# hmmlillian/Neural-Color-Transfer

Measured on AMD Instinct MI355X. Metric: 700x700 pairs/sec end-to-end L=5->1; PatchMatch HBM GB/s vs peak, higher is better.
Workload: dtype f32

## Files before the change

### neural-color-transfer_amd/csrc/k_wls_mg.hip

```cpp
#include "nct_internal.h"
#include <chrono>
#include <atomic>
#include <cstdlib>
#include <cstdio>
#include <cmath>
#include "nct_device.h"
#include <vector>
#include <cstring>
#include <string>
#include <thread>
#include <cstdarg>

namespace {
#ifndef NCT_MG_NS
#define NCT_MG_NS 3
#endif
constexpr int MG_NS = NCT_MG_NS;
static_assert(MG_NS >= 2 && MG_NS <= 4, "2, 3 or 4 smoothing sweeps per leg");
constexpr double MG_W[4] = {MG_NS == 2 ? 0.5808 : (MG_NS == 3 ? 0.5346 : 0.5193), MG_NS == 2 ? 2.6437 : (MG_NS == 3 ? 0.9677 : 0.7153), MG_NS == 3 ? 5.0974 : 1.5340, 8.0502};
constexpr double OMEGA = MG_W[0];
__host__ __device__ constexpr float mg_rk(int k) { return (float)(MG_W[k] / MG_W[0]); }
constexpr float MG_R0 = (float)(0.8 / MG_W[0]);
constexpr int NQMAX = 6;
#ifndef NCT_MG_TXB
#define NCT_MG_TXB 32
#define NCT_MG_TYB 16
#endif

typedef float vf;
struct Lvl { int H, W, n, nine;
             double *d, *wE, *wS, *wSE, *wSW, *pa, *pb;
             vf *fd, *fdinv, *fE, *fS, *fSE, *fSW;
             vf *fpst, *fpw;
             vf *b, *x, *x2;
             vf *lxm, *lxp, *lym, *lyp; };

struct PState { double gam[6], alp[6], bb[6]; int active[6]; int iters[6]; int nactive; int seq; double rho[6]; };

template <int NV>
__device__ __forceinline__ void mg_block_reduce(double (&v)[NV], double* __restrict__ partial, int lb = -1 ) {
    __shared__ double s_red[128 * NV];
    const int t = threadIdx.x;
    if (t >= 128) {
#pragma unroll
        for (int q = 0; q < NV; ++q) s_red[q * 128 + t - 128] = v[q];
    }
    __syncthreads();
    if (t < 128) {
#pragma unroll
        for (int q = 0; q < NV; ++q) v[q] += s_red[q * 128 + t];
    }
    __syncthreads();
    if (t >= 64 && t < 128) {
#pragma unroll
        for (int q = 0; q < NV; ++q) s_red[q * 128 + t - 64] = v[q];
    }
    __syncthreads();
    if (t < 64) {
#pragma unroll
        for (int q = 0; q < NV; ++q) {
            double x = v[q] + s_red[q * 128 + t];
            x += __shfl_down(x, 32); x += __shfl_down(x, 16); x += __shfl_down(x, 8);
            x += __shfl_down(x, 4); x += __shfl_down(x, 2); x += __shfl_down(x, 1);
            if (t == 0) partial[(size_t)(lb < 0 ? (int)blockIdx.x : lb) * NV + q] = x;
        }
    }
}
template <int NV>
__device__ __forceinline__ void mg_final_reduce(const double* __restrict__ partial, int nb, double (&out)[NV]) {
    __shared__ double s_fin[256 * NV];
    const int t = threadIdx.x;
    double acc[NV];
#pragma unroll
    for (int q = 0; q < NV; ++q) acc[q] = 0.0;
    for (int b = t; b < nb; b += 256)
#pragma unroll
        for (int q = 0; q < NV; ++q) acc[q] += partial[(size_t)b * NV + q];
#pragma unroll
    for (int q = 0; q < NV; ++q) s_fin[q * 256 + t] = acc[q];
    __syncthreads();
    for (int off = 128; off >= 1; off >>= 1) {
        if (t < off)
#pragma unroll
            for (int q = 0; q < NV; ++q) s_fin[q * 256 + t] += s_fin[q * 256 + t + off];
        __syncthreads();
    }
#pragma unroll
    for (int q = 0; q < NV; ++q) out[q] = s_fin[q * 256];
    __syncthreads();
}

template <int NV>
__device__ __forceinline__ void mg_final_reduce_strided(const double* __restrict__ partial, int nb, int stride, double (&out)[NV]) {
    __shared__ double s_fin2[256 * NV];
    const int t = threadIdx.x;
    double acc[NV];
#pragma unroll
    for (int q = 0; q < NV; ++q) acc[q] = 0.0;
    for (int b = t; b < nb; b += 256)
#pragma unroll
        for (int q = 0; q < NV; ++q) acc[q] += partial[(size_t)b * stride + q];
#pragma unroll
    for (int q = 0; q < NV; ++q) s_fin2[q * 256 + t] = acc[q];
    __syncthreads();
    for (int off = 128; off >= 1; off >>= 1) {
        if (t < off)
#pragma unroll
            for (int q = 0; q < NV; ++q) s_fin2[q * 256 + t] += s_fin2[q * 256 + t + off];
        __syncthreads();
    }
#pragma unroll
    for (int q = 0; q < NV; ++q) out[q] = s_fin2[q * 256];
    __syncthreads();
}

template <int NQ, typename F>
__device__ __forceinline__ void lvl_op(const Lvl& L, int i, F&& val , double (&y)[NQ]) {
    const int W = L.W, H = L.H;
    const int r = i / W, c = i - r * W;
    const double d = L.d[i];
    const bool e0 = c + 1 < W, e1 = c > 0, e2 = r + 1 < H, e3 = r > 0;
    const int j0 = e0 ? i + 1 : i, j1 = e1 ? i - 1 : i, j2 = e2 ? i + W : i, j3 = e3 ? i - W : i;
    const double w0 = L.wE[i], w1 = L.wE[j1], w2 = L.wS[i], w3 = L.wS[j3];
    double v0[NQ], v1[NQ], v2[NQ], v3[NQ];
#pragma unroll
    for (int q = 0; q < NQ; ++q) { y[q] = val(i, q); v0[q] = val(j0, q); v1[q] = val(j1, q); v2[q] = val(j2, q); v3[q] = val(j3, q); }
#pragma unroll
    for (int q = 0; q < NQ; ++q) {
        double t = d * y[q];
        t = e0 ? t - w0 * v0[q] : t;
        t = e1 ? t - w1 * v1[q] : t;
        t = e2 ? t - w2 * v2[q] : t;
        t = e3 ? t - w3 * v3[q] : t;
        y[q] = t;
    }
}

__device__ __forceinline__ int nb_dy(int k) { return k == 2 || k == 4 || k == 5 ? 1 : (k == 3 || k == 6 || k == 7 ? -1 : 0); }
__device__ __forceinline__ int nb_dx(int k) { return k == 0 || k == 4 || k == 6 ? 1 : (k == 1 || k == 5 || k == 7 ? -1 : 0); }
__device__ __forceinline__ unsigned nb_mask(const Lvl& L, int r, int c) {
    const bool xr = c + 1 < L.W, xl = c > 0, yd = r + 1 < L.H, yu = r > 0;
    unsigned m = (xr ? 1u : 0u) | (xl ? 2u : 0u) | (yd ? 4u : 0u) | (yu ? 8u : 0u);
    if (L.nine) m |= (xr && yd ? 16u : 0u) | (xl && yd ? 32u : 0u) | (xr && yu ? 64u : 0u) | (xl && yu ? 128u : 0u);
    return m;
}
__device__ __forceinline__ void coup8(const Lvl& L, int r, int c, double (&w)[8]) {
    const int W = L.W, i = r * W + c;
    const unsigned m = nb_mask(L, r, c);
    w[0] = (m & 1u) ? L.wE[i] : 0.0; w[1] = (m & 2u) ? L.wE[i - 1] : 0.0; w[2] = (m & 4u) ? L.wS[i] : 0.0; w[3] = (m & 8u) ? L.wS[i - W] : 0.0;
    w[4] = (m & 16u) ? L.wSE[i] : 0.0; w[5] = (m & 32u) ? L.wSW[i] : 0.0; w[6] = (m & 64u) ? L.wSW[i - W + 1] : 0.0; w[7] = (m & 128u) ? L.wSE[i - W - 1] : 0.0;
}
__global__ void k_mg_diag(Lvl L, const double* __restrict__ rough) {
    const int i = blockIdx.x * blockDim.x + threadIdx.x;
    if (i >= L.n) return;
    const int y = i / L.W, x = i - y * L.W;
    double a00 = 0.0;
    a00 += rough[i];
    if (x + 1 < L.W) a00 += L.wE[i];
    if (x > 0) a00 += L.wE[i - 1];
    if (y + 1 < L.H) a00 += L.wS[i];
    if (y > 0) a00 += L.wS[i - L.W];
    L.d[i] = a00;
    L.fd[i] = (vf)a00; L.fdinv[i] = (vf)(OMEGA / a00); L.fE[i] = (vf)L.wE[i]; L.fS[i] = (vf)L.wS[i];
}
__device__ __forceinline__ void mg_weights_at(const Lvl& L, int i) {
    const int r = i / L.W, c = i - r * L.W;
    double w[8]; coup8(L, r, c, w);
    const double d = L.d[i];
    double pa = 0.0, pb = 0.0;
    if (!(r & 1) && (c & 1)) { const double den = (d - w[2]) - w[3]; const bool e2 = c + 1 < L.W;
                               if (den > 0.0) { pa = ((w[1] + w[5]) + w[7]) / den; pb = ((w[0] + w[4]) + w[6]) / den; } else { pa = e2 ? 0.5 : 1.0; pb = e2 ? 0.5 : 0.0; } }
    else if ((r & 1) && !(c & 1)) { const double den = (d - w[0]) - w[1]; const bool e2 = r + 1 < L.H;
                                    if (den > 0.0) { pa = ((w[3] + w[6]) + w[7]) / den; pb = ((w[2] + w[4]) + w[5]) / den; } else { pa = e2 ? 0.5 : 1.0; pb = e2 ? 0.5 : 0.0; } }
    else if ((r & 1) && (c & 1)) pa = 1.0 / d;
    L.pa[i] = pa; L.pb[i] = pb;
}
__global__ void k_mg_weights(Lvl L) {
    const int i = blockIdx.x * blockDim.x + threadIdx.x;
    if (i >= L.n) return;
    mg_weights_at(L, i);
}
__device__ __forceinline__ void mg_pstencil_at(const Lvl& L, const Lvl& C, double* pst_out, int I) {
    const int Y = I / C.W, X = I - Y * C.W;
    const int W = L.W, H = L.H, r = 2 * Y, c = 2 * X, f = r * W + c;
    double pst[9];
#pragma unroll
    for (int k = 0; k < 9; ++k) pst[k] = 0.0;
    pst[4] = 1.0;
    if (c > 0) pst[3] = L.pb[f - 1];
    if (c + 1 < W) pst[5] = L.pa[f + 1];
    if (r > 0) pst[1] = L.pb[f - W];
    if (r + 1 < H) pst[7] = L.pa[f + W];
#pragma unroll
    for (int dy = -1; dy <= 1; dy += 2)
#pragma unroll
        for (int dx = -1; dx <= 1; dx += 2) {
            const int y = r + dy, x = c + dx;
            if (y < 0 || y >= H || x < 0 || x >= W) continue;
            double w[8]; coup8(L, y, x, w);
            const double wdiag = dy < 0 ? (dx < 0 ? w[4] : w[5]) : (dx < 0 ? w[6] : w[7]);
            const double wvert = dy < 0 ? w[2] : w[3];
            const double whor = dx < 0 ? w[0] : w[1];
            pst[(dy + 1) * 3 + dx + 1] = ((wdiag + wvert * pst[3 + dx + 1]) + whor * pst[(dy + 1) * 3 + 1]) * L.pa[y * W + x];
        }
#pragma unroll
    for (int k = 0; k < 9; ++k) { pst_out[(size_t)I * 9 + k] = pst[k]; L.fpst[(size_t)I * 9 + k] = (vf)pst[k]; }
}
__global__ void k_mg_pstencil(Lvl L, Lvl C, double* __restrict__ pst_out) {
    const int I = blockIdx.x * blockDim.x + threadIdx.x;
    if (I >= C.n) return;
    mg_pstencil_at(L, C, pst_out, I);
}
__device__ __forceinline__ void mg_pweights_at(const Lvl& L, const Lvl& C, int i) {
    const int r = i / L.W, c = i - r * L.W;
    const int Y0 = r >> 1, X0 = c >> 1, ny = (r & 1) ? 2 : 1, nx = (c & 1) ? 2 : 1;
    vf pw[4] = {0.f, 0.f, 0.f, 0.f};
    if (ny * nx > 1) {
        int sl = 0;
        for (int jy = 0; jy < ny; ++jy)
            for (int jx = 0; jx < nx; ++jx, ++sl) {
                const int Y = Y0 + jy, X = X0 + jx;
                if (Y < C.H && X < C.W) pw[sl] = L.fpst[(size_t)(Y * C.W + X) * 9 + (r - 2 * Y + 1) * 3 + (c - 2 * X + 1)];
            }
    }
#pragma unroll
    for (int k = 0; k < 4; ++k) L.fpw[(size_t)k * L.n + i] = pw[k];
}
__global__ void k_mg_pweights(Lvl L, Lvl C) {
    const int i = blockIdx.x * blockDim.x + threadIdx.x;
    if (i >= L.n) return;
    mg_pweights_at(L, C, i);
}
__device__ __forceinline__ void mg_galerkin_at(const Lvl& L, const Lvl& C, const double* pst, int I) {
    const int Wc = C.W, Hc = C.H, Y = I / Wc, X = I - Y * Wc;
    const int W = L.W, H = L.H;
    const int JY[5] = {0, 0, 1, 1, 1}, JX[5] = {0, 1, 0, 1, -1};
    bool jok[5]; double acc[5];
#pragma unroll
    for (int j = 0; j < 5; ++j) { const int yj = Y + JY[j], xj = X + JX[j]; jok[j] = yj < Hc && xj >= 0 && xj < Wc; acc[j] = 0.0; }
    const double* pI = pst + (size_t)I * 9;
    for (int dy = -1; dy <= 1; ++dy)
        for (int dx = -1; dx <= 1; ++dx) {
            const int y = 2 * Y + dy, x = 2 * X + dx;
            if (y < 0 || y >= H || x < 0 || x >= W) continue;
            const double pi = pI[(dy + 1) * 3 + dx + 1];
            double w[8]; coup8(L, y, x, w);
            const unsigned m = nb_mask(L, y, x);
            const double di = L.d[y * W + x];
#pragma unroll
            for (int j = 0; j < 5; ++j) {
                if (!jok[j]) continue;
                const double* pJ = pst + (size_t)(I + JY[j] * Wc + JX[j]) * 9;
                const int ry = dy - 2 * JY[j], rx = dx - 2 * JX[j];
                double au = (ry >= -1 && ry <= 1 && rx >= -1 && rx <= 1) ? di * pJ[(ry + 1) * 3 + rx + 1] : 0.0;
#pragma unroll
                for (int k = 0; k < 8; ++k) {
                    if (!(m & (1u << k))) continue;
                    const int ky = ry + nb_dy(k), kx = rx + nb_dx(k);
                    if (ky < -1 || ky > 1 || kx < -1 || kx > 1) continue;
                    au -= w[k] * pJ[(ky + 1) * 3 + kx + 1];
                }
                acc[j] += pi * au;
            }
        }
    C.d[I] = acc[0];
    C.wE[I] = jok[1] ? -acc[1] : 0.0;
    C.wS[I] = jok[2] ? -acc[2] : 0.0;
    C.wSE[I] = jok[3] ? -acc[3] : 0.0;
    C.wSW[I] = jok[4] ? -acc[4] : 0.0;
}
__global__ void k_mg_galerkin(Lvl L, Lvl C, const double* __restrict__ pst) {
    const int I = blockIdx.x * blockDim.x + threadIdx.x;
    if (I >= C.n) return;
    mg_galerkin_at(L, C, pst, I);
}
__device__ __forceinline__ void mg_finish_at(const Lvl& L, int i) {
    const int r = i / L.W, c = i - r * L.W;
    const double d = L.d[i];
    double w[8]; coup8(L, r, c, w);
    double s = fabs(d);
#pragma unroll
    for (int k = 0; k < 8; ++k) s += fabs(w[k]);
    const double h = 0.5 * s, dt = h > d ? h : d;
    L.fd[i] = (vf)d; L.fdinv[i] = (vf)(OMEGA / dt); L.fE[i] = (vf)L.wE[i]; L.fS[i] = (vf)L.wS[i]; L.fSE[i] = (vf)L.wSE[i]; L.fSW[i] = (vf)L.wSW[i];
}
__global__ void k_mg_finish(Lvl L) {
    const int i = blockIdx.x * blockDim.x + threadIdx.x;
    if (i >= L.n) return;
    mg_finish_at(L, i);
}

#ifndef NCT_MG_TAIL_N
#define NCT_MG_TAIL_N 512
#endif
constexpr int MG_TAIL_N = NCT_MG_TAIL_N;
constexpr int MG_MAXL = 12;
struct LvlPack { Lvl lv[MG_MAXL]; };
__global__ __launch_bounds__(1024) void k_mg_setup_tail(LvlPack P, int l0, int nl, double* pst) {
    const int t = threadIdx.x;
    for (int l = l0; l < nl; ++l) {
        const Lvl& L = P.lv[l - 1]; const Lvl& C = P.lv[l];
        for (int I = t; I < C.n; I += 1024) mg_pstencil_at(L, C, pst, I);
        __syncthreads();
        for (int i = t; i < L.n; i += 1024) mg_pweights_at(L, C, i);
        for (int I = t; I < C.n; I += 1024) mg_galerkin_at(L, C, pst, I);
        __syncthreads();
        for (int i = t; i < C.n; i += 1024) mg_finish_at(C, i);
        if (l + 1 < nl) {
            for (int i = t; i < C.n; i += 1024) mg_weights_at(C, i);
        }
        __syncthreads();
    }
}

struct PxCoef { vf d, dinv, w[8]; unsigned ex; };
template <bool NINE>
__device__ __forceinline__ PxCoef px_coef(const Lvl& L, int gy, int gx) {
    const int i = gy * L.W + gx, W = L.W;
    PxCoef c;
    const bool xr = gx + 1 < W, xl = gx > 0, yd = gy + 1 < L.H, yu = gy > 0;
    c.ex = (xr ? 1u : 0u) | (xl ? 2u : 0u) | (yd ? 4u : 0u) | (yu ? 8u : 0u);
    c.d = L.fd[i]; c.dinv = L.fdinv[i];
    c.w[0] = xr ? L.fE[i] : 0.f; c.w[1] = xl ? L.fE[i - 1] : 0.f; c.w[2] = yd ? L.fS[i] : 0.f; c.w[3] = yu ? L.fS[i - W] : 0.f;
    if (NINE) {
        c.ex |= (xr && yd ? 16u : 0u) | (xl && yd ? 32u : 0u) | (xr && yu ? 64u : 0u) | (xl && yu ? 128u : 0u);
        c.w[4] = (xr && yd) ? L.fSE[i] : 0.f; c.w[5] = (xl && yd) ? L.fSW[i] : 0.f; c.w[6] = (xr && yu) ? L.fSW[i - W + 1] : 0.f; c.w[7] = (xl && yu) ? L.fSE[i - W - 1] : 0.f;
    } else { c.w[4] = c.w[5] = c.w[6] = c.w[7] = 0.f; }
    return c;
}
template <int LW> __device__ __forceinline__ constexpr int lds_off(int k) {
    return k == 0 ? 1 : k == 1 ? -1 : k == 2 ? LW : k == 3 ? -LW : k == 4 ? LW + 1 : k == 5 ? LW - 1 : k == 6 ? -LW + 1 : -LW - 1;
}
template <int NQ, int LW, int LN, bool NINE>
__device__ __forceinline__ void lds_op(const PxCoef& c, const vf* __restrict__ s_v, int p, const vf (&own)[NQ], vf (&y)[NQ]) {
#pragma unroll
    for (int q = 0; q < NQ; ++q) y[q] = c.d * own[q];
#pragma unroll
    for (int k = 0; k < (NINE ? 8 : 4); ++k)
        if (c.ex & (1u << k)) {
#pragma unroll
            for (int q = 0; q < NQ; ++q) y[q] -= c.w[k] * s_v[q * LN + p + lds_off<LW>(k)];
        }
}
__device__ __forceinline__ int mg_tile_of_block(int bid, int ntiles) {
    const int q = ntiles >> 3, r = ntiles & 7, xcd = bid & 7, idx = bid >> 3;
    return (xcd < r ? xcd * (q + 1) : r * (q + 1) + (xcd - r) * q) + idx;
}
constexpr int mg_threads(int TX, int TY, bool X0 = false) { return ((TX + 2 * MG_NS + 1 + (X0 ? 2 : 0)) * (TY + 2 * MG_NS + 1 + (X0 ? 2 : 0)) + 63) / 64 * 64; }
template <int NQ, int TX, int TY, typename TB, bool NINE, bool X0 = false>
__global__ __launch_bounds__(mg_threads(TX, TY, X0)) void k_mg_down(const PState* __restrict__ st, Lvl F, const TB* __restrict__ b, vf* __restrict__ x, Lvl C, vf* __restrict__ bc, const vf* __restrict__ x1 = nullptr) {
    const int nact = st->nactive;
    constexpr int S0 = X0 ? 1 : 0;
    constexpr int HA = MG_NS + 1 + S0, HB = MG_NS + S0, LW = TX + HA + HB, LH = TY + HA + HB, LN = LW * LH;
    static_assert(LN <= mg_threads(TX, TY, X0) && mg_threads(TX, TY, X0) <= 1024, "one thread per pixel of the tile and its halo");
    __shared__ vf s_a[NQ * LN], s_b[NQ * LN];
    const int tiles_x = (F.W + TX - 1) / TX, tile = mg_tile_of_block(blockIdx.x, gridDim.x);
    const int x0 = (tile % tiles_x) * TX, y0 = (tile / tiles_x) * TY;
    const int p = threadIdx.x;
    const int ly = p / LW, lx = p - ly * LW;
    const int gy = y0 + ly - HA, gx = x0 + lx - HA;
    const bool valid = p < LN && gy >= 0 && gy < F.H && gx >= 0 && gx < F.W;
    auto ring = [&](int k) { return valid && lx >= k && lx <= LW - 1 - k && ly >= k && ly <= LH - 1 - k; };
    const bool interior = valid && lx >= HA && lx < HA + TX && ly >= HA && ly < HA + TY;
    const bool coarse = interior && !(gy & 1) && !(gx & 1);
    const int i = gy * F.W + gx;
    vf bq[NQ], xk[NQ], ps[9]; PxCoef c;
    if (valid) {
        c = px_coef<NINE>(F, gy, gx);
        if (coarse) {
            const vf* pp = F.fpst + (size_t)((gy >> 1) * C.W + (gx >> 1)) * 9;
#pragma unroll
            for (int k = 0; k < 9; ++k) ps[k] = pp[k];
        }
#pragma unroll
        for (int q = 0; q < NQ; ++q) { bq[q] = (vf)b[(size_t)q * F.n + i]; xk[q] = X0 ? x1[(size_t)q * F.n + i] : bq[q] * c.dinv; s_a[q * LN + p] = xk[q]; }
    }
    if (nact == 0) return;
    __syncthreads();
#pragma unroll
    for (int k = 1 - S0; k < MG_NS; ++k) {
        vf* src = ((k + S0) & 1) ? s_a : s_b; vf* dst = ((k + S0) & 1) ? s_b : s_a;
        if (ring(k + S0)) {
            vf y[NQ]; lds_op<NQ, LW, LN, NINE>(c, src, p, xk, y);
#pragma unroll
            for (int q = 0; q < NQ; ++q) {
                xk[q] = xk[q] + (bq[q] - y[q]) * (k == 0 ? c.dinv : c.dinv * mg_rk(k));
                dst[q * LN + p] = xk[q];
                if (k == MG_NS - 1 && interior) x[(size_t)q * F.n + i] = xk[q];
            }
        }
        __syncthreads();
    }
    vf* xs = ((MG_NS + S0) & 1) ? s_a : s_b; vf* rs = ((MG_NS + S0) & 1) ? s_b : s_a;
    if (ring(MG_NS + S0)) {
        vf yv[NQ]; lds_op<NQ, LW, LN, NINE>(c, xs, p, xk, yv);
#pragma unroll
        for (int q = 0; q < NQ; ++q) rs[q * LN + p] = bq[q] - yv[q];
    }
    __syncthreads();
    if (coarse) {
        const bool xr = (c.ex & 1u) != 0, xl = (c.ex & 2u) != 0, yd = (c.ex & 4u) != 0, yu = (c.ex & 8u) != 0;
        const bool in[9] = {xl && yu, yu, xr && yu, xl, true, xr, xl && yd, yd, xr && yd};
        vf acc[NQ];
#pragma unroll
        for (int q = 0; q < NQ; ++q) acc[q] = 0.0f;
#pragma unroll
        for (int k = 0; k < 9; ++k)
            if (in[k]) {
#pragma unroll
                for (int q = 0; q < NQ; ++q) acc[q] += ps[k] * rs[q * LN + p + (k / 3 - 1) * LW + (k % 3 - 1)];
            }
#pragma unroll
        for (int q = 0; q < NQ; ++q) bc[(size_t)q * C.n + (gy >> 1) * C.W + (gx >> 1)] = acc[q];
    }
}
template <int NQ, int TX, int TY, typename TB, bool NINE>
__global__ __launch_bounds__(mg_threads(TX, TY)) void k_mg_up(const PState* __restrict__ st, Lvl L, const TB* __restrict__ b, const vf* __restrict__ x, int Wc, int nc,
                                                              const vf* __restrict__ ec, vf* __restrict__ xo) {
    const int nact = st->nactive;
    constexpr bool ODD = (MG_NS & 1) != 0;
    constexpr int HA = ODD ? MG_NS + 1 : MG_NS, HB = ODD ? MG_NS : MG_NS + 1, LW = TX + HA + HB, LH = TY + HA + HB, LN = LW * LH;
    constexpr int OL = ODD ? 1 : 0, OR = ODD ? 0 : 1;
    __shared__ vf s_a[NQ * LN], s_b[NQ * LN];
    const int tiles_x = (L.W + TX - 1) / TX, tile = mg_tile_of_block(blockIdx.x, gridDim.x);
    const int x0 = (tile % tiles_x) * TX, y0 = (tile / tiles_x) * TY;
    const int p = threadIdx.x;
    const int ly = p / LW, lx = p - ly * LW;
    const int gy = y0 + ly - HA, gx = x0 + lx - HA;
    const bool valid = p < LN && gy >= 0 && gy < L.H && gx >= 0 && gx < L.W;
    auto ring = [&](int k) { return valid && lx >= OL + k && lx <= LW - 1 - OR - k && ly >= OL + k && ly <= LH - 1 - OR - k; };
    const bool oy = (gy & 1) != 0, ox = (gx & 1) != 0;
    const int i = gy * L.W + gx;
    vf bq[NQ], xk[NQ], pw[4]; PxCoef c;
    if (valid) {
        c = px_coef<NINE>(L, gy, gx);
#pragma unroll
        for (int k = 0; k < 4; ++k) pw[k] = L.fpw[(size_t)k * L.n + i];
#pragma unroll
        for (int q = 0; q < NQ; ++q) { bq[q] = (vf)b[(size_t)q * L.n + i]; xk[q] = x[(size_t)q * L.n + i]; }
        if (!oy && !ox) {
            const int ip = (gy >> 1) * Wc + (gx >> 1);
#pragma unroll
            for (int q = 0; q < NQ; ++q) s_a[q * LN + p] = ec[(size_t)q * nc + ip];
        }
    }
    if (nact == 0) return;
    __syncthreads();
    if (ring(0)) {
        const bool xr = (c.ex & 1u) != 0, yd = (c.ex & 4u) != 0;
        const int o0 = -(oy ? LW : 0) - (ox ? 1 : 0);
        const int o1 = (oy && ox) ? -LW + 1 : (ox ? 1 : LW);
        const bool e1 = (oy && ox) ? xr : (ox ? xr : yd);
        const bool e2 = oy && ox && yd, e3 = oy && ox && yd && xr;
        const bool copy = !oy && !ox;
        const int a1 = e1 ? o1 : o0, a2 = e2 ? LW - 1 : o0, a3 = e3 ? LW + 1 : o0;
        vf v0[NQ], v1[NQ], v2[NQ], v3[NQ];
#pragma unroll
        for (int q = 0; q < NQ; ++q) { v0[q] = s_a[q * LN + p + (copy ? 0 : o0)]; v1[q] = s_a[q * LN + p + (copy ? 0 : a1)]; v2[q] = s_a[q * LN + p + (copy ? 0 : a2)]; v3[q] = s_a[q * LN + p + (copy ? 0 : a3)]; }
#pragma unroll
        for (int q = 0; q < NQ; ++q) {
            vf e = pw[0] * v0[q];
            e = e1 ? e + pw[1] * v1[q] : e;
            e = e2 ? e + pw[2] * v2[q] : e;
            e = e3 ? e + pw[3] * v3[q] : e;
            e = copy ? v0[q] : e;
            xk[q] = xk[q] + e; s_b[q * LN + p] = xk[q];
        }
    }
    __syncthreads();
#pragma unroll
    for (int k = 0; k < MG_NS; ++k) {
        vf* src = (k & 1) ? s_a : s_b; vf* dst = (k & 1) ? s_b : s_a;
        if (ring(k + 1)) {
            vf y[NQ]; lds_op<NQ, LW, LN, NINE>(c, src, p, xk, y);
#pragma unroll
            for (int q = 0; q < NQ; ++q) {
                xk[q] = xk[q] + (bq[q] - y[q]) * (k == 0 ? c.dinv : c.dinv * mg_rk(k));
                if (k == MG_NS - 1) xo[(size_t)q * L.n + i] = xk[q]; else dst[q * LN + p] = xk[q];
            }
        }
        if (k < MG_NS - 1) __syncthreads();
    }
}
constexpr int LBX = 32, LBY = 16, LBP = LBX + 1, LBN = LBY * LBP + 1;
constexpr float LINE_OM = 0.9f;
__global__ void k_mg_lines_setup(Lvl L) {
    const int t = blockIdx.x * blockDim.x + threadIdx.x;
    const int W = L.W, H = L.H, nbx = (W + LBX - 1) / LBX, nby = (H + LBY - 1) / LBY;
    if (t < H * nbx) {
        const int r = t / nbx, c0 = (t - r * nbx) * LBX;
        double p = 0.0;
        for (int c = c0; c < W && c < c0 + LBX; ++c) {
            const int i = r * W + c;
            if (c == c0) { p = L.d[i]; L.lxm[i] = 0.0f; }
            else { const double w = L.wE[i - 1], m = w / p; p = L.d[i] - w * m; L.lxm[i] = (vf)m; }
            L.lxp[i] = (vf)(1.0 / p);
        }
    } else if (t < H * nbx + W * nby) {
        const int u = t - H * nbx, c = u / nby, r0 = (u - c * nby) * LBY;
        double p = 0.0;
        for (int r = r0; r < H && r < r0 + LBY; ++r) {
            const int i = r * W + c;
            if (r == r0) { p = L.d[i]; L.lym[i] = 0.0f; }
            else { const double w = L.wS[i - W], m = w / p; p = L.d[i] - w * m; L.lym[i] = (vf)m; }
            L.lyp[i] = (vf)(1.0 / p);
        }
    }
}
template <int LEN, int STR>
__device__ __forceinline__ void line_solve(const vf* __restrict__ s_r, vf* __restrict__ s_e, const vf* __restrict__ s_m, const vf* __restrict__ s_p, const vf* __restrict__ s_w, int len) {
    vf y[LEN];
    if (len == LEN) {
        constexpr int CH = 8;
        static_assert(LEN % CH == 0, "line length");
#pragma unroll
        for (int k = 0; k < LEN; ++k) y[k] = s_r[k * STR];
        vf t = 0.0f;
#pragma unroll
        for (int k0 = 0; k0 < LEN; k0 += CH) {
            vf m[CH];
#pragma unroll
            for (int j = 0; j < CH; ++j) m[j] = s_m[(k0 + j) * STR];
#pragma unroll
            for (int j = 0; j < CH; ++j) { const int k = k0 + j; if (k == 0) t = y[0]; else { t = y[k] + m[j] * t; y[k] = t; } }
        }
#pragma unroll
        for (int k0 = LEN - CH; k0 >= 0; k0 -= CH) {
            vf pp[CH], ww[CH];
#pragma unroll
            for (int j = 0; j < CH; ++j) { pp[j] = s_p[(k0 + j) * STR]; ww[j] = s_w[(k0 + j) * STR]; }
#pragma unroll
            for (int j = CH - 1; j >= 0; --j) { const int k = k0 + j; t = k == LEN - 1 ? y[k] * pp[j] : (y[k] + ww[j] * t) * pp[j]; y[k] = t; }
        }
#pragma unroll
        for (int k = 0; k < LEN; ++k) s_e[k * STR] = y[k];
        return;
    }
#pragma unroll
    for (int k = 0; k < LEN; ++k) if (k < len) y[k] = s_r[k * STR];
    vf t = y[0];
#pragma unroll
    for (int k = 1; k < LEN; ++k) if (k < len) { t = y[k] + s_m[k * STR] * t; y[k] = t; }
#pragma unroll
    for (int k = LEN - 1; k >= 0; --k)
        if (k < len) {
            if (k == len - 1) t = y[k] * s_p[k * STR];
            else t = (y[k] + s_w[k * STR] * t) * s_p[k * STR];
            s_e[k * STR] = t;
        }
}
template <int NQ, bool POST>
__global__ __launch_bounds__(LBX * LBY, 8) void k_mg_block(const PState* __restrict__ st, Lvl L, const vf* __restrict__ b, const vf* __restrict__ xin, vf* __restrict__ xout) {
    const int nact = st->nactive;
    constexpr int XW = LBX + 2, XN = XW * (LBY + 2);
    static_assert(NQ * XN <= (NQ + 6) * LBN, "the halo tile of the iterate lives where e1 and the factors go afterwards");
    __shared__ vf s_all[(2 * NQ + 6) * LBN];
    vf* const s_r = s_all; vf* const s_e1 = s_all + NQ * LBN; vf* const s_x = s_e1;
    vf* const s_xm = s_all + 2 * NQ * LBN; vf* const s_xp = s_xm + LBN; vf* const s_xw = s_xp + LBN; vf* const s_ym = s_xw + LBN; vf* const s_yp = s_ym + LBN; vf* const s_yw = s_yp + LBN;
    const int W = L.W, H = L.H, nbx = (W + LBX - 1) / LBX;
    const int blk = mg_tile_of_block(blockIdx.x, gridDim.x);
    const int x0 = (blk % nbx) * LBX, y0 = (blk / nbx) * LBY;
    const int bw = x0 + LBX <= W ? LBX : W - x0, bh = y0 + LBY <= H ? LBY : H - y0;
    const int p = threadIdx.x, ly = p / LBX, lx = p - ly * LBX, gy = y0 + ly, gx = x0 + lx;
    const bool valid = ly < bh && lx < bw;
    const int i = gy * W + gx, lp = ly * LBP + lx;
    vf own[NQ], bq[NQ];
    if (POST) {
        for (int h = p; h < XN; h += LBX * LBY) {
            const int hy = h / XW, hx = h - hy * XW, yy = y0 + hy - 1, xx = x0 + hx - 1;
            if (yy >= 0 && yy < H && xx >= 0 && xx < W) {
#pragma unroll
                for (int q = 0; q < NQ; ++q) s_x[q * XN + h] = xin[(size_t)q * L.n + yy * W + xx];
            }
        }
    }
    vf fE_own = 0.f, fS_own = 0.f, c_xm = 0.f, c_xp = 0.f, c_ym = 0.f, c_yp = 0.f;
    if (valid) {
        c_xm = L.lxm[i]; c_xp = L.lxp[i]; c_ym = L.lym[i]; c_yp = L.lyp[i]; fE_own = L.fE[i]; fS_own = L.fS[i];
#pragma unroll
        for (int q = 0; q < NQ; ++q) bq[q] = b[(size_t)q * L.n + i];
    }
    if (nact == 0) return;
    if (POST) {
        __syncthreads();
        if (valid) {
            const vf d = L.fd[i];
            const bool xr = gx + 1 < W, xl = gx > 0, yd = gy + 1 < H, yu = gy > 0;
            const vf wW = xl ? L.fE[i - 1] : 0.f, wN = yu ? L.fS[i - W] : 0.f;
            const int hp = (ly + 1) * XW + lx + 1;
#pragma unroll
            for (int q = 0; q < NQ; ++q) {
                own[q] = s_x[q * XN + hp];
                const vf vE = s_x[q * XN + hp + 1], vW = s_x[q * XN + hp - 1], vS = s_x[q * XN + hp + XW], vN = s_x[q * XN + hp - XW];
                vf y = d * own[q];
                y = xr ? y - fE_own * vE : y;
                y = xl ? y - wW * vW : y;
                y = yd ? y - fS_own * vS : y;
                y = yu ? y - wN * vN : y;
                bq[q] = bq[q] - y;
            }
        }
        __syncthreads();
    }
    if (valid) {
        s_xm[lp] = c_xm; s_xp[lp] = c_xp; s_ym[lp] = c_ym; s_yp[lp] = c_yp; s_xw[lp] = fE_own; s_yw[lp] = fS_own;
#pragma unroll
        for (int q = 0; q < NQ; ++q) s_r[q * LBN + lp] = bq[q];
    }
    __syncthreads();
    if (!POST) { if (p < LBY * NQ) { const int row = p % LBY, q = p / LBY; if (row < bh) { const int o = row * LBP; line_solve<LBX, 1>(s_r + q * LBN + o, s_e1 + q * LBN + o, s_xm + o, s_xp + o, s_xw + o, bw); } } }
    else       { if (p < LBX * NQ) { const int col = p % LBX, q = p / LBX; if (col < bw) line_solve<LBY, LBP>(s_r + q * LBN + col, s_e1 + q * LBN + col, s_ym + col, s_yp + col, s_yw + col, bh); } }
    __syncthreads();
    if (valid) {
#pragma unroll
        for (int q = 0; q < NQ; ++q) {
            vf acc = 0.0f;
            if (!POST) { if (ly + 1 < bh) acc += fS_own * s_e1[q * LBN + lp + LBP]; if (ly > 0) acc += s_yw[lp - LBP] * s_e1[q * LBN + lp - LBP]; }
            else       { if (lx + 1 < bw) acc += fE_own * s_e1[q * LBN + lp + 1];   if (lx > 0) acc += s_xw[lp - 1] * s_e1[q * LBN + lp - 1]; }
            s_r[q * LBN + lp] = acc;
        }
    }
    __syncthreads();
    if (!POST) { if (p < LBX * NQ) { const int col = p % LBX, q = p / LBX; if (col < bw) line_solve<LBY, LBP>(s_r + q * LBN + col, s_r + q * LBN + col, s_ym + col, s_yp + col, s_yw + col, bh); } }
    else       { if (p < LBY * NQ) { const int row = p % LBY, q = p / LBY; if (row < bh) { const int o = row * LBP; line_solve<LBX, 1>(s_r + q * LBN + o, s_r + q * LBN + o, s_xm + o, s_xp + o, s_xw + o, bw); } } }
    __syncthreads();
    if (valid) {
#pragma unroll
        for (int q = 0; q < NQ; ++q) {
            const vf u = (s_e1[q * LBN + lp] + s_r[q * LBN + lp]) * LINE_OM;
            xout[(size_t)q * L.n + i] = POST ? own[q] + u : u;
        }
    }
}

#ifndef NCT_MID_MAXP0
#define NCT_MID_MAXP0 2
#endif
static_assert(NCT_MID_MAXP0 == 1 || NCT_MID_MAXP0 == 2, "k_mg_mid is instantiated for one or two pixels per thread at its first level (four measured slower: DESIGN.md 9)");
constexpr int MID_T = 1024, MID_P1 = 1, MID_N1 = MID_T * MID_P1, MID_LV = 5;
constexpr int mid_cap(int d) { return d == 1 ? 1024 : (d == 2 ? 256 : 64); }
constexpr int mid_stash_off(int d) { return d <= 1 ? 0 : mid_stash_off(d - 1) + 14 * mid_cap(d - 1); }
constexpr int MID_STASH = mid_stash_off(MID_LV);
constexpr int mid_ppt(int P0, int D) { return D == 0 ? P0 : (D == 1 ? MID_P1 : 1); }
struct MidPack { Lvl lv[MID_LV]; int nl; };
__device__ __forceinline__ vf mid_op(const PxCoef& c, const vf* __restrict__ s_v, int i, int W, vf* centre = nullptr) {
    const vf v0 = s_v[i];
    if (centre) *centre = v0;
    vf y = c.d * v0;
    vf t[8];
#pragma unroll
    for (int k = 0; k < 8; ++k) t[k] = s_v[(c.ex & (1u << k)) ? i + nb_dy(k) * W + nb_dx(k) : i];
#pragma unroll
    for (int k = 0; k < 8; ++k) y -= c.w[k] * ((c.ex & (1u << k)) ? t[k] : 0.0f);
    return y;
}
__device__ __forceinline__ vf mid_restrict(const vf* __restrict__ s_res, const vf (&ps)[9], int I, int Wc, int Wf, int Hf) {
    const int Y = I / Wc, X = I - Y * Wc, r = 2 * Y, c = 2 * X;
    vf acc = 0.0f, t[9]; bool in[9];
#pragma unroll
    for (int k = 0; k < 9; ++k) {
        const int yy = r + k / 3 - 1, xx = c + k % 3 - 1;
        in[k] = yy >= 0 && yy < Hf && xx >= 0 && xx < Wf;
        t[k] = s_res[in[k] ? yy * Wf + xx : r * Wf + c];
    }
#pragma unroll
    for (int k = 0; k < 9; ++k) acc = in[k] ? acc + ps[k] * t[k] : acc;
    return acc;
}
__device__ __forceinline__ vf mid_prolong(const vf* __restrict__ s_c, const vf (&pw)[4], int gy, int gx, int Wc, int Hc) {
    const int Y0 = gy >> 1, X0 = gx >> 1;
    const bool oy = (gy & 1) != 0, ox = (gx & 1) != 0;
    const bool xr = X0 + 1 < Wc, yd = Y0 + 1 < Hc;
    const int i00 = Y0 * Wc + X0, i01 = xr ? i00 + 1 : i00, i10 = yd ? i00 + Wc : i00, i11 = (yd && xr) ? i00 + Wc + 1 : i00;
    const vf c00 = s_c[i00], c01 = s_c[i01], c10 = s_c[i10], c11 = s_c[i11];
    if (!oy && !ox) return c00;
    vf e = pw[0] * c00;
    if (oy && ox) {
        e = xr ? e + pw[1] * c01 : e;
        e = yd ? e + pw[2] * c10 : e;
        e = (yd && xr) ? e + pw[3] * c11 : e;
    } else if (ox) { e = xr ? e + pw[1] * c01 : e; }
    else { e = yd ? e + pw[1] * c10 : e; }
    return e;
}
template <int P0, int D>
__device__ __forceinline__ void mid_level(const MidPack& P, int q, int t, vf* __restrict__ sA, vf* __restrict__ sB, vf* __restrict__ sC, vf* __restrict__ sS,
                                          const vf (&breg)[mid_ppt(P0, D)], int sweeps) {
    constexpr int PPT = mid_ppt(P0, D);
    const Lvl& L = P.lv[D];
    const int n = L.n, W = L.W;
    if (D == P.nl - 1) {
        if (t < n) sA[t] = breg[0];
        __syncthreads();
        if (t < 64) {
            const int i = t;
            const bool live = i < n;
            const int r = live ? i / W : 0, c = live ? i - r * W : 0;
            vf bq = 0.f, d = 0.f, dv = 0.f, w[8]; unsigned ex = 0;
#pragma unroll
            for (int k = 0; k < 8; ++k) w[k] = 0.f;
            if (live) { const PxCoef pc = px_coef<true>(L, r, c); d = pc.d; dv = pc.dinv; ex = pc.ex; bq = sA[i];
#pragma unroll
                for (int k = 0; k < 8; ++k) w[k] = pc.w[k]; }
            vf x = 0.0f;
            for (int s = 0; s < sweeps; ++s) {
                vf y = d * x;
#pragma unroll
                for (int k = 0; k < 8; ++k) {
                    const vf xn = __shfl(x, (i + nb_dy(k) * W + nb_dx(k)) & 63);
                    if (ex & (1u << k)) y -= w[k] * xn;
                }
                if (live) x = x + (bq - y) * (dv * MG_R0);
            }
            if (live) { if (D == 0) L.x2[(size_t)q * n + i] = x; else sC[i] = x; }
        }
        __syncthreads();
        return;
    }
    if constexpr (D + 1 < MID_LV) {
        const Lvl& C = P.lv[D + 1];
        constexpr int CPT = mid_ppt(P0, D + 1);
        vf* __restrict__ stash = sS + mid_stash_off(D);
        vf x[PPT];
        {
            PxCoef c[PPT]; vf ps[CPT][9];
#pragma unroll
            for (int k = 0; k < PPT; ++k) { const int i = t + k * MID_T; if (i < n) c[k] = px_coef<true>(L, i / W, i % W); }
#pragma unroll
            for (int k = 0; k < CPT; ++k) { const int I = t + k * MID_T; if (I < C.n) {
#pragma unroll
                for (int j = 0; j < 9; ++j) ps[k][j] = L.fpst[(size_t)I * 9 + j]; } }
            if constexpr (D >= 1) {
                if (t < n) {
                    vf pw[4];
#pragma unroll
                    for (int j = 0; j < 4; ++j) pw[j] = L.fpw[(size_t)j * n + t];
                    stash[t] = c[0].d; stash[n + t] = c[0].dinv;
#pragma unroll
                    for (int j = 0; j < 8; ++j) stash[(2 + j) * n + t] = c[0].w[j];
#pragma unroll
                    for (int j = 0; j < 4; ++j) stash[(10 + j) * n + t] = pw[j];
                }
            }
#pragma unroll
            for (int k = 0; k < PPT; ++k) { const int i = t + k * MID_T; if (i < n) sA[i] = breg[k] * c[k].dinv; }
            __syncthreads();
#pragma unroll
            for (int sw = 1; sw < MG_NS; ++sw) {
                vf* src = (sw & 1) ? sA : sB; vf* dst = (sw & 1) ? sB : sA;
#pragma unroll
                for (int k = 0; k < PPT; ++k) {
                    const int i = t + k * MID_T;
                    if (i < n) {
                        vf xs; const vf y = mid_op(c[k], src, i, W, &xs);
                        const vf xv = xs + (breg[k] - y) * (c[k].dinv * mg_rk(sw));
                        dst[i] = xv;
                        if (sw == MG_NS - 1) x[k] = xv;
                    }
                }
                __syncthreads();
            }
            {
                vf* xs = (MG_NS & 1) ? sA : sB; vf* rs = (MG_NS & 1) ? sB : sA;
#pragma unroll
                for (int k = 0; k < PPT; ++k) { const int i = t + k * MID_T; if (i < n) rs[i] = breg[k] - mid_op(c[k], xs, i, W); }
            }
            __syncthreads();
            vf bc[CPT];
#pragma unroll
            for (int k = 0; k < CPT; ++k) { const int I = t + k * MID_T; bc[k] = I < C.n ? mid_restrict((MG_NS & 1) ? sB : sA, ps[k], I, C.W, W, L.H) : 0.f; }
            __syncthreads();
            asm volatile("" ::: "memory");
            mid_level<P0, D + 1>(P, q, t, sA, sB, sC, sS, bc, sweeps);
        }
        PxCoef c[PPT]; vf pw[PPT][4];
        if constexpr (D == 0) {
#pragma unroll
            for (int k = 0; k < PPT; ++k) { const int i = t + k * MID_T; if (i < n) { c[k] = px_coef<true>(L, i / W, i % W);
#pragma unroll
                for (int j = 0; j < 4; ++j) pw[k][j] = L.fpw[(size_t)j * n + i]; } }
        } else {
            if (t < n) {
                const int gy = t / W, gx = t - gy * W;
                const bool xr = gx + 1 < W, xl = gx > 0, yd = gy + 1 < L.H, yu = gy > 0;
                c[0].ex = (xr ? 1u : 0u) | (xl ? 2u : 0u) | (yd ? 4u : 0u) | (yu ? 8u : 0u) | (xr && yd ? 16u : 0u) | (xl && yd ? 32u : 0u) | (xr && yu ? 64u : 0u) | (xl && yu ? 128u : 0u);
                c[0].d = stash[t]; c[0].dinv = stash[n + t];
#pragma unroll
                for (int j = 0; j < 8; ++j) c[0].w[j] = stash[(2 + j) * n + t];
#pragma unroll
                for (int j = 0; j < 4; ++j) pw[0][j] = stash[(10 + j) * n + t];
            }
        }
#pragma unroll
        for (int k = 0; k < PPT; ++k) {
            const int i = t + k * MID_T;
            if (i < n) sA[i] = x[k] + mid_prolong(sC, pw[k], i / W, i % W, C.W, C.H);
        }
        __syncthreads();
#pragma unroll
        for (int sw = 0; sw < MG_NS; ++sw) {
            vf* src = (sw & 1) ? sB : sA; vf* dst = (sw & 1) ? sA : sB;
#pragma unroll
            for (int k = 0; k < PPT; ++k) {
                const int i = t + k * MID_T;
                if (i < n) {
                    vf xs; const vf y = mid_op(c[k], src, i, W, &xs);
                    const vf v = xs + (breg[k] - y) * (sw == 0 ? c[k].dinv : c[k].dinv * mg_rk(sw));
                    if (sw < MG_NS - 1) dst[i] = v;
                    else if (D == 0) L.x2[(size_t)q * n + i] = v; else sC[i] = v;
                }
            }
            __syncthreads();
        }
    }
}
template <int P0>
__global__ __launch_bounds__(MID_T) void k_mg_mid(const PState* __restrict__ st, MidPack P, int sweeps) {
    const int nact = st->nactive;
    __shared__ vf sA[MID_T * P0], sB[MID_T * P0], sC[MID_N1], sS[MID_STASH];
    const int q = blockIdx.x, t = threadIdx.x;
    const Lvl& L0 = P.lv[0];
    vf b[P0];
#pragma unroll
    for (int k = 0; k < P0; ++k) { const int i = t + k * MID_T; b[k] = i < L0.n ? L0.b[(size_t)q * L0.n + i] : 0.f; }
    if (nact == 0) return;
    mid_level<P0, 0>(P, q, t, sA, sB, sC, sS, b, sweeps);
}


__device__ __forceinline__ void pcg_publish(PState* __restrict__ host_out, const PState& v, int seq) {
    PState o = v; o.seq = 0;
    *host_out = o;
    __threadfence_system();
    __hip_atomic_store(&host_out->seq, seq, __ATOMIC_RELEASE, __HIP_MEMORY_SCOPE_SYSTEM);
}
template <int NQ>
__global__ __launch_bounds__(256) void k_pcg_start(Lvl L, const double* __restrict__ rough, const double* __restrict__ X , double* __restrict__ x6, double* __restrict__ r, vf* __restrict__ rf, double* __restrict__ partial) {
    const int i = blockIdx.x * 256 + threadIdx.x;
    double acc[2 * NQ];
#pragma unroll
    for (int q = 0; q < 2 * NQ; ++q) acc[q] = 0.0;
    if (i < L.n) {
        auto xv = [&](int j, int q) { return X[((size_t)(q / 3) * L.n + j) * 3 + (q % 3)]; };
        double y[NQ]; lvl_op<NQ>(L, i, xv, y);
        const double rg = rough[i];
#pragma unroll
        for (int q = 0; q < NQ; ++q) {
            const double x0 = xv(i, q);
            const double bq = rg * x0;
            const double rv = bq - y[q];
            x6[(size_t)q * L.n + i] = x0; r[(size_t)q * L.n + i] = rv; rf[(size_t)q * L.n + i] = (vf)rv;
            acc[q] = rv * rv; acc[NQ + q] = bq * bq;
        }
    }
    mg_block_reduce<2 * NQ>(acc, partial);
}
template <int NQ>
__global__ void k_pcg_start_fin(const double* __restrict__ partial, int nb, PState* __restrict__ st, double rtol2, PState* __restrict__ host_out, int seq) {
    double s[2 * NQ]; mg_final_reduce<2 * NQ>(partial, nb, s);
    if (threadIdx.x < NQ) { const int q = threadIdx.x; st->bb[q] = s[NQ + q]; st->gam[q] = 0; st->alp[q] = 0; st->iters[q] = 0; st->rho[q] = s[q];
                            st->active[q] = (s[q] > rtol2 * s[NQ + q]) ? 1 : 0; }
    __syncthreads();
    if (threadIdx.x == 0) { int na = 0; for (int q = 0; q < NQ; ++q) na += st->active[q]; st->nactive = na; if (host_out) pcg_publish(host_out, *st, seq); }
}
template <int NQ>
__global__ __launch_bounds__(256) void k_cg_apply(const PState* __restrict__ st, Lvl L, const vf* __restrict__ z, const double* __restrict__ r,
                                                  double* __restrict__ w, double* __restrict__ partial) {
    const int nact = st->nactive;
    const int lb = mg_tile_of_block(blockIdx.x, gridDim.x);
    const int i = lb * 256 + threadIdx.x;
    double acc[3 * NQ];
#pragma unroll
    for (int q = 0; q < 3 * NQ; ++q) acc[q] = 0.0;
    auto uv = [&](int j, int q) { return (double)z[(size_t)q * L.n + j]; };
    double y[NQ], rq[NQ], uq[NQ];
#pragma unroll
    for (int q = 0; q < NQ; ++q) { y[q] = 0.0; rq[q] = 0.0; uq[q] = 0.0; }
    if (i < L.n) {
        lvl_op<NQ>(L, i, uv, y);
#pragma unroll
        for (int q = 0; q < NQ; ++q) { rq[q] = r[(size_t)q * L.n + i]; uq[q] = uv(i, q); }
    }
    if (nact == 0) return;
    if (i < L.n) {
#pragma unroll
        for (int q = 0; q < NQ; ++q) {
            const double u = uq[q], rv = rq[q];
            w[(size_t)q * L.n + i] = y[q];
            acc[q] = rv * u; acc[NQ + q] = y[q] * u; acc[2 * NQ + q] = rv * rv;
        }
    }
    mg_block_reduce<3 * NQ>(acc, partial, lb);
}
template <int NQ>
__global__ void k_cg_fin(const PState* __restrict__ st, const double* __restrict__ partial, int nb, double* __restrict__ sums) {
    if (st->nactive == 0) return;
    double s[NQ]; mg_final_reduce_strided<NQ>(partial + blockIdx.x * NQ, nb, 3 * NQ, s);
    if (threadIdx.x < NQ) sums[blockIdx.x * NQ + threadIdx.x] = s[threadIdx.x];
}
template <int NQ>
__global__ __launch_bounds__(256) void k_cg_update(int n, const PState* __restrict__ sc, PState* __restrict__ sn, const double* __restrict__ sums, double rtol2, int first,
                                                   const vf* __restrict__ z, const double* __restrict__ w, double* __restrict__ p, double* __restrict__ s,
                                                   double* __restrict__ x, double* __restrict__ r, vf* __restrict__ rf, PState* __restrict__ host_out, int seq) {
    if (sc->nactive == 0) { if (blockIdx.x == 0 && threadIdx.x == 0) { *sn = *sc; if (host_out) pcg_publish(host_out, *sc, seq); } return; }
    double al[NQ], be[NQ]; bool act[NQ];
#pragma unroll
    for (int q = 0; q < NQ; ++q) {
        const double gam = sums[q], del = sums[NQ + q], rho = sums[2 * NQ + q];
        act[q] = sc->active[q] != 0 && rho > rtol2 * sc->bb[q];
        be[q] = first ? 0.0 : gam / sc->gam[q];
        al[q] = first ? gam / del : gam / (del - be[q] * gam / sc->alp[q]);
    }
    if (blockIdx.x == 0 && threadIdx.x == 0) {
        int na = 0;
#pragma unroll
        for (int q = 0; q < NQ; ++q) {
            sn->bb[q] = sc->bb[q];
            sn->gam[q] = act[q] ? sums[q] : sc->gam[q]; sn->alp[q] = act[q] ? al[q] : sc->alp[q];
            sn->iters[q] = sc->iters[q] + (act[q] ? 1 : 0); sn->active[q] = act[q] ? 1 : 0; na += act[q] ? 1 : 0;
            sn->rho[q] = sc->active[q] != 0 ? sums[2 * NQ + q] : sc->rho[q];
        }
        sn->nactive = na;
        if (host_out) pcg_publish(host_out, *sn, seq);
    }
    const int i = blockIdx.x * 256 + threadIdx.x;
    if (i >= n) return;
    vf zq[NQ]; double wq[NQ], pq[NQ], sq[NQ], xq[NQ], rq[NQ];
#pragma unroll
    for (int q = 0; q < NQ; ++q) {
        zq[q] = 0.f; wq[q] = pq[q] = sq[q] = xq[q] = rq[q] = 0.0;
        if (act[q]) {
            const size_t j = (size_t)q * n + i;
            zq[q] = z[j]; wq[q] = w[j]; xq[q] = x[j]; rq[q] = r[j];
            if (!first) { pq[q] = p[j]; sq[q] = s[j]; }
        }
    }
#pragma unroll
    for (int q = 0; q < NQ; ++q) {
        if (!act[q]) continue;
        const size_t j = (size_t)q * n + i;
        const double zv = (double)zq[q], wv = wq[q];
        const double pn = first ? zv : zv + be[q] * pq[q];
        const double sv = first ? wv : wv + be[q] * sq[q];
        p[j] = pn; s[j] = sv;
        x[j] = xq[q] + al[q] * pn;
        const double rn = rq[q] - al[q] * sv;
        r[j] = rn; rf[j] = (vf)rn;
    }
}
template <int NQ>
__global__ void k_pcg_finish(int n, const double* __restrict__ x6, double* __restrict__ X) {
    const int i = blockIdx.x * blockDim.x + threadIdx.x;
    if (i >= n * NQ) return;
    const int q = i / n, px = i - q * n;
    X[((size_t)(q / 3) * n + px) * 3 + (q % 3)] = x6[i];
}
}

#define LCHK() NCT_LAUNCH_CHECK()
#ifndef NCT_WLS_BATCH
#define NCT_WLS_BATCH 2
#endif

namespace {
struct ErrSink {
    std::string err;
    int fail(int code, const char* fmt, ...) { char buf[512]; va_list ap; va_start(ap, fmt); vsnprintf(buf, sizeof buf, fmt, ap); va_end(ap); err = buf; return code; }
};
static std::atomic<int> g_seq{0};
struct PartBufs {
    double *x6, *r, *p, *sv, *w, *partial, *sums; PState* st;
    vf* rf;
    std::vector<Lvl> lv;
    PState* hst;
    const double* rough;
    nct_ctx* kt;
    int maxit;
    bool trace;
    bool forecast;
    bool lines;
    int iters[NQMAX];
};
template <int NQ>
int pcg_part(ErrSink* ctx, hipStream_t s, double* X , PartBufs& B, double rtol) {
    const std::vector<Lvl>& lv = B.lv;
    const int nl = (int)lv.size();
    const Lvl& F = lv[0];
    const int N = F.n, nb = cdiv(N, 256);
    double *x6 = B.x6, *r = B.r, *p = B.p, *sv = B.sv, *w = B.w, *partial = B.partial, *sums = B.sums;
    vf* rf = B.rf;
    PState* st = B.st;
    const PState* cur = st;
    const double rtol2 = rtol * rtol;
    hipLaunchKernelGGL(k_pcg_start<NQ>, dim3(nb), dim3(256), 0, s, F, B.rough, (const double*)X, (double*)x6, (double*)r, rf, (double*)partial); LCHK();
    int seq_of_slot[2] = {0, 0};
    seq_of_slot[0] = ++g_seq;
    hipLaunchKernelGGL(k_pcg_start_fin<NQ>, dim3(1), dim3(256), 0, s, (const double*)partial, nb, st, rtol2, &B.hst[0], seq_of_slot[0]); LCHK();

    constexpr int TXB = NCT_MG_TXB, TYB = NCT_MG_TYB;
    auto down = [&](int l) {
        const dim3 gb(cdiv(lv[l].W, TXB) * cdiv(lv[l].H, TYB)), gs(cdiv(lv[l].W, 16) * cdiv(lv[l].H, 8));
        if (l == 0 && B.lines) {
            constexpr int TYL = TYB - 2;
            const dim3 gbl(cdiv(lv[0].W, TXB) * cdiv(lv[0].H, TYL));
            if (lv[l].n >= 100000) hipLaunchKernelGGL((k_mg_down<NQ, TXB, TYL, vf, false, true>), gbl, dim3(mg_threads(TXB, TYL, true)), 0, s, cur, lv[l], (const vf*)rf, lv[l].x, lv[l + 1], lv[l + 1].b, (const vf*)lv[0].x2);
            else                   hipLaunchKernelGGL((k_mg_down<NQ, 16, 8, vf, false, true>), gs, dim3(mg_threads(16, 8, true)), 0, s, cur, lv[l], (const vf*)rf, lv[l].x, lv[l + 1], lv[l + 1].b, (const vf*)lv[0].x2);
        } else if (l == 0) {
            if (lv[l].n >= 100000) hipLaunchKernelGGL((k_mg_down<NQ, TXB, TYB, vf, false>), gb, dim3(mg_threads(TXB, TYB)), 0, s, cur, lv[l], (const vf*)rf, lv[l].x, lv[l + 1], lv[l + 1].b);
            else                   hipLaunchKernelGGL((k_mg_down<NQ, 16, 8, vf, false>), gs, dim3(mg_threads(16, 8)), 0, s, cur, lv[l], (const vf*)rf, lv[l].x, lv[l + 1], lv[l + 1].b);
        } else {
            if (lv[l].n >= 100000) hipLaunchKernelGGL((k_mg_down<NQ, TXB, TYB, vf, true>), gb, dim3(mg_threads(TXB, TYB)), 0, s, cur, lv[l], (const vf*)lv[l].b, lv[l].x, lv[l + 1], lv[l + 1].b);
            else                   hipLaunchKernelGGL((k_mg_down<NQ, 16, 8, vf, true>), gs, dim3(mg_threads(16, 8)), 0, s, cur, lv[l], (const vf*)lv[l].b, lv[l].x, lv[l + 1], lv[l + 1].b);
        }
    };
    auto block_step = [&](bool post) {
        if (!B.lines) return;
        const dim3 gl(cdiv(lv[0].W, LBX) * cdiv(lv[0].H, LBY));
        if (!post) hipLaunchKernelGGL((k_mg_block<NQ, false>), gl, dim3(LBX * LBY), 0, s, cur, lv[0], (const vf*)rf, (const vf*)nullptr, lv[0].x2);
        else       hipLaunchKernelGGL((k_mg_block<NQ, true>), gl, dim3(LBX * LBY), 0, s, cur, lv[0], (const vf*)rf, (const vf*)lv[0].x2, lv[0].x);
    };
    auto up = [&](int l, const vf* ec) {
        const dim3 gb(cdiv(lv[l].W, TXB) * cdiv(lv[l].H, TYB)), gs(cdiv(lv[l].W, 16) * cdiv(lv[l].H, 8));
        const int Wc = lv[l + 1].W, nc = lv[l + 1].n;
        if (l == 0) {
            if (lv[l].n >= 100000) hipLaunchKernelGGL((k_mg_up<NQ, TXB, TYB, vf, false>), gb, dim3(mg_threads(TXB, TYB)), 0, s, cur, lv[l], (const vf*)rf, (const vf*)lv[l].x, Wc, nc, ec, lv[l].x2);
            else                   hipLaunchKernelGGL((k_mg_up<NQ, 16, 8, vf, false>), gs, dim3(mg_threads(16, 8)), 0, s, cur, lv[l], (const vf*)rf, (const vf*)lv[l].x, Wc, nc, ec, lv[l].x2);
        } else {
            if (lv[l].n >= 100000) hipLaunchKernelGGL((k_mg_up<NQ, TXB, TYB, vf, true>), gb, dim3(mg_threads(TXB, TYB)), 0, s, cur, lv[l], (const vf*)lv[l].b, (const vf*)lv[l].x, Wc, nc, ec, lv[l].x2);
            else                   hipLaunchKernelGGL((k_mg_up<NQ, 16, 8, vf, true>), gs, dim3(mg_threads(16, 8)), 0, s, cur, lv[l], (const vf*)lv[l].b, (const vf*)lv[l].x, Wc, nc, ec, lv[l].x2);
        }
    };
    int tail0 = nl - 1;
    auto mid_fits = [&](int first) {
        if (nl - first > MID_LV) return false;
        for (int l = first; l < nl; ++l) { const int d = l - first; if (lv[l].n > (d == 0 ? NCT_MID_MAXP0 * MID_T : mid_cap(d))) return false; }
        return true;
    };
    while (tail0 > 1 && mid_fits(tail0 - 1)) --tail0;
    MidPack pack; memset(&pack, 0, sizeof pack); pack.nl = nl - tail0;
    for (int l = tail0; l < nl; ++l) pack.lv[l - tail0] = lv[l];
    bool ktime = false;
    auto kt_b = [&](int id) -> int { if (ktime && B.kt->kt_begin(s, id)) return ctx->fail(NCT_ERR_HIP, "%s", B.kt->err.c_str()); return 0; };
    auto kt_e = [&]() -> int { if (ktime && B.kt->kt_end(s)) return ctx->fail(NCT_ERR_HIP, "%s", B.kt->err.c_str()); return 0; };
    auto vcycle = [&]() -> int {
        if (ktime) {
            if (B.lines) { NCT_TRY(kt_b(NCT_KT_WLS_BLOCK_PRE)); block_step(false); LCHK(); NCT_TRY(kt_e()); }
            NCT_TRY(kt_b(NCT_KT_WLS_DOWN)); down(0); LCHK(); NCT_TRY(kt_e());
            NCT_TRY(kt_b(NCT_KT_WLS_COARSE));
            for (int l = 1; l < tail0; ++l) { down(l); LCHK(); }
            if (lv[tail0].n <= MID_T) hipLaunchKernelGGL(k_mg_mid<1>, dim3(NQ), dim3(MID_T), 0, s, cur, pack, 60);
            else                      hipLaunchKernelGGL(k_mg_mid<2>, dim3(NQ), dim3(MID_T), 0, s, cur, pack, 60);
            LCHK();
            for (int l = tail0 - 1; l >= 1; --l) { up(l, lv[l + 1].x2); LCHK(); }
            NCT_TRY(kt_e());
            NCT_TRY(kt_b(NCT_KT_WLS_UP)); up(0, lv[1].x2); LCHK(); NCT_TRY(kt_e());
            if (B.lines) { NCT_TRY(kt_b(NCT_KT_WLS_BLOCK_POST)); block_step(true); LCHK(); NCT_TRY(kt_e()); }
            return 0;
        }
        block_step(false); LCHK();
        for (int l = 0; l < tail0; ++l) { down(l); LCHK(); }
        if (lv[tail0].n <= MID_T) hipLaunchKernelGGL(k_mg_mid<1>, dim3(NQ), dim3(MID_T), 0, s, cur, pack, 60);
        else                      hipLaunchKernelGGL(k_mg_mid<2>, dim3(NQ), dim3(MID_T), 0, s, cur, pack, 60);
        LCHK();
        for (int l = tail0 - 1; l >= 0; --l) { up(l, lv[l + 1].x2); LCHK(); }
        block_step(true); LCHK();
        return 0;
    };
    const vf* z = B.lines ? lv[0].x : lv[0].x2;
    const int maxit = B.maxit, batch = NCT_WLS_BATCH;
    PState* hst = B.hst;
    PState* pub_to = nullptr; int pub_seq = 0;
    auto iteration = [&](int it) -> int {
        cur = st + (it & 1);
        PState* nxt = st + ((it + 1) & 1);
        ktime = B.kt != nullptr && it >= 2 && it < 6 && tail0 >= 1;
        NCT_TRY(vcycle());
        NCT_TRY(kt_b(NCT_KT_WLS_APPLY));
        hipLaunchKernelGGL(k_cg_apply<NQ>, dim3(nb), dim3(256), 0, s, cur, F, z, (const double*)r, (double*)w, (double*)partial); LCHK();
        NCT_TRY(kt_e());
        hipLaunchKernelGGL(k_cg_fin<NQ>, dim3(3), dim3(256), 0, s, cur, (const double*)partial, nb, (double*)sums); LCHK();
        NCT_TRY(kt_b(NCT_KT_WLS_UPDATE));
        hipLaunchKernelGGL(k_cg_update<NQ>, dim3(nb), dim3(256), 0, s, N, cur, nxt, (const double*)sums, rtol2, it == 0 ? 1 : 0, z, (const double*)w,
                           (double*)p, (double*)sv, (double*)x6, (double*)r, rf, pub_to, pub_seq); LCHK();
        NCT_TRY(kt_e());
        cur = nxt;
        return 0;
    };
    auto wait_published = [&](int slot) -> int {
        const int want_seq = seq_of_slot[slot];
        const auto t0 = std::chrono::steady_clock::now();
        for (unsigned spins = 1; __atomic_load_n(&hst[slot].seq, __ATOMIC_ACQUIRE) != want_seq; ++spins) {
            if (spins > 4096) std::this_thread::yield();
            if ((spins & 0xFFFFu) == 0) {
                const hipError_t q = hipStreamQuery(s);
                if (q != hipSuccess && q != hipErrorNotReady) return ctx->fail(NCT_ERR_HIP, "WLS MG-PCG: stream error while polling the solver state: %s", hipGetErrorString(q));
                if (std::chrono::steady_clock::now() - t0 > std::chrono::seconds(60)) return ctx->fail(NCT_ERR_HIP, "WLS MG-PCG: the solver state was not published within 60 s");
            }
        }
        return 0;
    };
    int it = 0; bool done = false;
    int issued = 0, seen = -1;
    int its_at_snapshot[2] = {0, 0};
    PState fin; memset(&fin, 0, sizeof fin);
    double prev_rho[6]; int prev_its = -1;
    int remaining_after_seen = -1;
    int its_seen = 0;
    bool forecast_on = B.forecast;
    while (true) {
        int want = batch;
        if (forecast_on && remaining_after_seen >= 0) {
            const int inflight = it - its_seen;
            want = remaining_after_seen - inflight;
            if (want > batch) want = batch;
            if (want < 0) want = 0;
            if (want == 0 && issued == seen) { want = batch; forecast_on = false; }
        }
        if (it + want > maxit) want = maxit - it;
        if (want > 0) {
            for (int k = 0; k < want; ++k, ++it) {
                if (k == want - 1) { seq_of_slot[(issued + 1) & 1] = ++g_seq; pub_to = &hst[(issued + 1) & 1]; pub_seq = seq_of_slot[(issued + 1) & 1]; }
                int rc = iteration(it); pub_to = nullptr; if (rc) return rc;
            }
            ++issued; its_at_snapshot[issued & 1] = it;
        }
        if (seen == issued) break;
        ++seen;
        NCT_TRY(wait_published(seen & 1));
        fin = hst[seen & 1];
        its_seen = its_at_snapshot[seen & 1];
        if (fin.nactive == 0) { done = true; break; }
        if (it >= maxit && seen == issued) break;
        if (B.forecast) {
            const int ridx = its_seen > 0 ? its_seen - 1 : 0;
            int need = -1; bool ok = prev_its >= 0 && ridx > prev_its;
            if (ok) {
                need = 1;
                for (int q = 0; q < NQ; ++q) {
                    if (!fin.active[q]) continue;
                    const double thr = rtol2 * fin.bb[q], rho = fin.rho[q];
                    if (!(rho > 0.0) || !(prev_rho[q] > 0.0) || !(thr > 0.0)) { ok = false; break; }
                    const double decay = pow(rho / prev_rho[q], 1.0 / (double)(ridx - prev_its));
                    if (!(decay < 0.95)) { ok = false; break; }
                    const double m = rho * decay <= thr ? 1.0 : 1.0 + ceil(log(thr / (rho * decay)) / log(decay));
                    if (m > need) need = (int)(m < 1e6 ? m : 1e6);
                }
            }
            remaining_after_seen = ok ? need : -1;
            for (int q = 0; q < NQ; ++q) prev_rho[q] = fin.rho[q];
            prev_its = ridx;
        }
    }
    if (!done) return ctx->fail(NCT_ERR_HIP, "WLS MG-PCG did not converge in %d iterations", maxit);
    hipLaunchKernelGGL(k_pcg_finish<NQ>, dim3(cdiv(N * NQ, 256)), dim3(256), 0, s, N, (const double*)x6, X); LCHK();
    for (int q = 0; q < NQ; ++q) B.iters[q] = fin.iters[q];
    if (B.trace) {
        int mx = 0; for (int q = 0; q < NQ; ++q) mx = fin.iters[q] > mx ? fin.iters[q] : mx;
        fprintf(stderr, "nct wls: %d x %d, %d iterations enqueued, %d needed (+1 that finds every system converged), %d snapshots read\n", F.W, F.H, it, mx, seen + 1);
    }
    return 0;
}
}

int nctk_wls_solve_mg(nct_ctx* ctx, hipStream_t s, double* X, const double* rough, const double* wx, const double* wy, int H, int W,
                      double rtol, int* iters_out ) {
    const bool split = ctx->wls_split != 0;
    const int nq0 = split ? 3 : 6;
    std::vector<Lvl> lv;
    std::vector<void*> owned;
    struct Cleanup { nct_ctx* c; std::vector<void*>& v; ~Cleanup() { for (void* q : v) c->release(q); } } cleanup{ctx, owned};
    auto newd = [&](size_t n) -> double* { void* q = ctx->alloc(n * sizeof(double)); if (q) owned.push_back(q); return (double*)q; };
    auto newf = [&](size_t n) -> vf* { void* q = ctx->alloc(n * sizeof(vf)); if (q) owned.push_back(q); return (vf*)q; };
    {
        int h = H, w = W;
        for (int l = 0;; ++l) {
            Lvl L; memset(&L, 0, sizeof L); L.H = h; L.W = w; L.n = h * w; L.nine = l > 0 ? 1 : 0;
            const bool last = L.n <= 64 || (h <= 8 && w <= 8) || l >= 15;
            if (l == 0) { L.wE = (double*)wx; L.wS = (double*)wy; }
            else { L.wE = newd(L.n); L.wS = newd(L.n); L.wSE = newd(L.n); L.wSW = newd(L.n); L.fSE = newf(L.n); L.fSW = newf(L.n);
                   if (!L.wE || !L.wS || !L.wSE || !L.wSW || !L.fSE || !L.fSW) return NCT_ERR_HIP; }
            L.d = newd(L.n); L.fd = newf(L.n); L.fdinv = newf(L.n); L.fE = newf(L.n); L.fS = newf(L.n);
            if (!last) { L.pa = newd(L.n); L.pb = newd(L.n); }
            if (!last) { L.fpst = newf((size_t)((h + 1) / 2) * ((w + 1) / 2) * 9); L.fpw = newf((size_t)L.n * 4); }
            L.b = l == 0 ? nullptr : newf((size_t)L.n * nq0); L.x = newf((size_t)L.n * nq0); L.x2 = newf((size_t)L.n * nq0);
            if (l == 0 && ctx->wls_lines) { L.lxm = newf(L.n); L.lxp = newf(L.n); L.lym = newf(L.n); L.lyp = newf(L.n); if (!L.lxm || !L.lxp || !L.lym || !L.lyp) return NCT_ERR_HIP; }
            if (!L.d || !L.fd || !L.fdinv || !L.fE || !L.fS || (!last && (!L.pa || !L.pb || !L.fpst || !L.fpw)) || (l > 0 && !L.b) || !L.x || !L.x2) return NCT_ERR_HIP;
            lv.push_back(L);
            if (last) break;
            h = (h + 1) / 2; w = (w + 1) / 2;
        }
        if (lv.back().n > 64 || lv.size() < 2) return ctx->fail(NCT_ERR_INVALID, "wls: unsupported grid %dx%d (coarsest level %d)", W, H, lv.back().n);
    }
    const int nl = (int)lv.size();
    {
        double* pst = newd((size_t)lv[1].n * 9);
        if (!pst) return NCT_ERR_HIP;
        hipLaunchKernelGGL(k_mg_diag, dim3(cdiv(lv[0].n, 256)), dim3(256), 0, s, lv[0], rough); LCHK();
        if (ctx->wls_lines) { hipLaunchKernelGGL(k_mg_lines_setup, dim3(cdiv(lv[0].H * cdiv(lv[0].W, LBX) + lv[0].W * cdiv(lv[0].H, LBY), 128)), dim3(128), 0, s, lv[0]); LCHK(); }
        int l_tail = nl;
        for (int l = 1; l < nl; ++l) if (lv[l].n <= MG_TAIL_N) { l_tail = l; break; }
        if (nl > MG_MAXL) l_tail = nl;
        for (int l = 0; l < l_tail; ++l) {
            const dim3 g(cdiv(lv[l].n, 256));
            if (l > 0) {
                const dim3 gc(cdiv(lv[l].n, 128));
                hipLaunchKernelGGL(k_mg_pstencil, gc, dim3(128), 0, s, lv[l - 1], lv[l], pst); LCHK();
                hipLaunchKernelGGL(k_mg_pweights, dim3(cdiv(lv[l - 1].n, 256)), dim3(256), 0, s, lv[l - 1], lv[l]); LCHK();
                hipLaunchKernelGGL(k_mg_galerkin, gc, dim3(128), 0, s, lv[l - 1], lv[l], (const double*)pst); LCHK();
                hipLaunchKernelGGL(k_mg_finish, g, dim3(256), 0, s, lv[l]); LCHK();
            }
            if (l + 1 < nl) { hipLaunchKernelGGL(k_mg_weights, g, dim3(256), 0, s, lv[l]); LCHK(); }
        }
        if (l_tail < nl) {
            LvlPack P;
            for (int l = 0; l < nl; ++l) P.lv[l] = lv[l];
            hipLaunchKernelGGL(k_mg_setup_tail, dim3(1), dim3(1024), 0, s, P, l_tail, nl, pst); LCHK();
        }
    }
    const int N = lv[0].n, nb = cdiv(N, 256);
    static_assert(4 * sizeof(PState) <= 4096, "pinned read-back area too small");
    PartBufs part[2];
    const int nparts = split ? 2 : 1;
    for (int h = 0; h < nparts; ++h) {
        PartBufs& B = part[h];
        const size_t v = (size_t)N * nq0;
        B.rf = newf(v); if (!B.rf) return NCT_ERR_HIP;
        B.x6 = newd(v); B.r = newd(v); B.p = newd(v); B.sv = newd(v); B.w = newd(v); B.partial = newd((size_t)nb * 3 * nq0); B.sums = newd(3 * nq0);
        B.st = (PState*)ctx->alloc(2 * sizeof(PState)); if (B.st) owned.push_back(B.st);
        if (!B.x6 || !B.r || !B.p || !B.sv || !B.w || !B.partial || !B.sums || !B.st) return NCT_ERR_HIP;
        B.lv = lv;
        if (h == 1) for (int l = 0; l < nl; ++l) {
            Lvl& L = B.lv[l];
            L.b = l == 0 ? nullptr : newf((size_t)L.n * nq0); L.x = newf((size_t)L.n * nq0); L.x2 = newf((size_t)L.n * nq0);
            if ((l > 0 && !L.b) || !L.x || !L.x2) return NCT_ERR_HIP;
        }
        B.hst = (PState*)ctx->pinned + 2 * h;
        B.maxit = ctx->wls_maxit; B.forecast = ctx->wls_forecast != 0; B.lines = ctx->wls_lines != 0; B.trace = getenv("NCT_WLS_TRACE") != nullptr; B.rough = rough; B.kt = (ctx->kt_on && !split) ? ctx : nullptr;
        memset(B.iters, 0, sizeof B.iters);
    }
    if (!split) {
        ErrSink sink;
        const int rc = pcg_part<6>(&sink, s, X, part[0], rtol);
        if (rc) return ctx->fail(rc, "%s", sink.err.c_str());
        if (iters_out) for (int q = 0; q < 6; ++q) iters_out[q] = part[0].iters[q];
        return 0;
    }
    hipStream_t s2 = ctx->stream_wls;
    NCT_HIP(hipEventRecord(ctx->ev_wls_fork, s));
    NCT_HIP(hipStreamWaitEvent(s2, ctx->ev_wls_fork, 0));
    ErrSink sink_a, sink_b;
    int rc_b = 0;
    const int dev = ctx->device;
    std::thread helper([&] {
        if (hipSetDevice(dev) != hipSuccess) { rc_b = sink_b.fail(NCT_ERR_HIP, "hipSetDevice failed on the WLS helper thread"); return; }
        rc_b = pcg_part<3>(&sink_b, s2, X + (size_t)3 * N, part[1], rtol);
    });
    const int rc_a = pcg_part<3>(&sink_a, s, X, part[0], rtol);
    helper.join();
    hipError_t e1 = hipEventRecord(ctx->ev_wls_join, s2), e2 = hipStreamWaitEvent(s, ctx->ev_wls_join, 0);
    if (rc_a) return ctx->fail(rc_a, "%s", sink_a.err.c_str());
    if (rc_b) return ctx->fail(rc_b, "%s", sink_b.err.c_str());
    NCT_HIP(e1); NCT_HIP(e2);
    if (iters_out) for (int q = 0; q < 3; ++q) { iters_out[q] = part[0].iters[q]; iters_out[3 + q] = part[1].iters[q]; }
    return 0;
}
```

Measured before the change: 15.73.

## Skip converged systems in multigrid legs and test residual after the CG update

The multigrid down, up and block-smoother kernels now build a mask of still-active systems and run their smoothing legs only over those channels, dispatching on the active count at compile time so LDS and register work scale with it. The CG update computes the new residual norm itself, and a new single-block kernel decides convergence from it. This lets a system stop one iteration earlier and removes the rho term from the earlier reduction. The cost is an extra small kernel launch per iteration and more template instantiations, which increase code size.

```diff
diff --git a/neural-color-transfer_amd/csrc/k_wls_mg.hip b/neural-color-transfer_amd/csrc/k_wls_mg.hip
--- a/neural-color-transfer_amd/csrc/k_wls_mg.hip
+++ b/neural-color-transfer_amd/csrc/k_wls_mg.hip
@@ -37,6 +37,26 @@
 
 struct PState { double gam[6], alp[6], bb[6]; int active[6]; int iters[6]; int nactive; int seq; double rho[6]; };
 
+template <int NQ> __device__ __forceinline__ void act_load(const PState* __restrict__ st, int (&a)[NQ]) {
+#pragma unroll
+    for (int q = 0; q < NQ; ++q) a[q] = st->active[q];
+}
+template <int NQ> __device__ __forceinline__ unsigned act_mask(const int (&a)[NQ]) {
+    unsigned m = 0;
+#pragma unroll
+    for (int q = 0; q < NQ; ++q) m |= a[q] != 0 ? 1u << q : 0u;
+    return m;
+}
+template <int NQ> __device__ __forceinline__ void act_list(unsigned m, int (&qm)[NQ]) {
+#pragma unroll
+    for (int j = 0; j < NQ; ++j) { qm[j] = m ? __builtin_ctz(m) : 0; m &= m - 1u; }
+}
+template <int N> struct ActCount { static constexpr int value = N; };
+template <int NQ, int K = NQ, typename Fn> __device__ __forceinline__ void act_dispatch(int na, Fn&& f) {
+    if (na == K) f(ActCount<K>{});
+    else if constexpr (K > 1) act_dispatch<NQ, K - 1>(na, f);
+}
+
 template <int NV>
 __device__ __forceinline__ void mg_block_reduce(double (&v)[NV], double* __restrict__ partial, int lb = -1 ) {
     __shared__ double s_red[128 * NV];
@@ -91,7 +111,7 @@
 }
 
 template <int NV>
-__device__ __forceinline__ void mg_final_reduce_strided(const double* __restrict__ partial, int nb, int stride, double (&out)[NV]) {
+__device__ __forceinline__ void mg_final_reduce_strided(const double* __restrict__ partial, int nb, int stride, double (&out)[NV], const int* act = nullptr) {
     __shared__ double s_fin2[256 * NV];
     const int t = threadIdx.x;
     double acc[NV];
@@ -99,7 +119,7 @@
     for (int q = 0; q < NV; ++q) acc[q] = 0.0;
     for (int b = t; b < nb; b += 256)
 #pragma unroll
-        for (int q = 0; q < NV; ++q) acc[q] += partial[(size_t)b * stride + q];
+        for (int q = 0; q < NV; ++q) if (act == nullptr || act[q]) acc[q] += partial[(size_t)b * stride + q];
 #pragma unroll
     for (int q = 0; q < NV; ++q) s_fin2[q * 256 + t] = acc[q];
     __syncthreads();
@@ -115,7 +135,7 @@
 }
 
 template <int NQ, typename F>
-__device__ __forceinline__ void lvl_op(const Lvl& L, int i, F&& val , double (&y)[NQ]) {
+__device__ __forceinline__ void lvl_op(const Lvl& L, int i, F&& val , double (&y)[NQ], const int* act = nullptr) {
     const int W = L.W, H = L.H;
     const int r = i / W, c = i - r * W;
     const double d = L.d[i];
@@ -124,9 +144,13 @@
     const double w0 = L.wE[i], w1 = L.wE[j1], w2 = L.wS[i], w3 = L.wS[j3];
     double v0[NQ], v1[NQ], v2[NQ], v3[NQ];
 #pragma unroll
-    for (int q = 0; q < NQ; ++q) { y[q] = val(i, q); v0[q] = val(j0, q); v1[q] = val(j1, q); v2[q] = val(j2, q); v3[q] = val(j3, q); }
-#pragma unroll
     for (int q = 0; q < NQ; ++q) {
+        v0[q] = v1[q] = v2[q] = v3[q] = 0.0;
+        if (act == nullptr || act[q]) { y[q] = val(i, q); v0[q] = val(j0, q); v1[q] = val(j1, q); v2[q] = val(j2, q); v3[q] = val(j3, q); }
+    }
+#pragma unroll
+    for (int q = 0; q < NQ; ++q) {
+        if (act != nullptr && !act[q]) continue;
         double t = d * y[q];
         t = e0 ? t - w0 * v0[q] : t;
         t = e1 ? t - w1 * v1[q] : t;
@@ -349,7 +373,7 @@
 constexpr int mg_threads(int TX, int TY, bool X0 = false) { return ((TX + 2 * MG_NS + 1 + (X0 ? 2 : 0)) * (TY + 2 * MG_NS + 1 + (X0 ? 2 : 0)) + 63) / 64 * 64; }
 template <int NQ, int TX, int TY, typename TB, bool NINE, bool X0 = false>
 __global__ __launch_bounds__(mg_threads(TX, TY, X0)) void k_mg_down(const PState* __restrict__ st, Lvl F, const TB* __restrict__ b, vf* __restrict__ x, Lvl C, vf* __restrict__ bc, const vf* __restrict__ x1 = nullptr) {
-    const int nact = st->nactive;
+    int abit[NQ]; act_load<NQ>(st, abit);
     constexpr int S0 = X0 ? 1 : 0;
     constexpr int HA = MG_NS + 1 + S0, HB = MG_NS + S0, LW = TX + HA + HB, LH = TY + HA + HB, LN = LW * LH;
     static_assert(LN <= mg_threads(TX, TY, X0) && mg_threads(TX, TY, X0) <= 1024, "one thread per pixel of the tile and its halo");
@@ -364,7 +388,7 @@
     const bool interior = valid && lx >= HA && lx < HA + TX && ly >= HA && ly < HA + TY;
     const bool coarse = interior && !(gy & 1) && !(gx & 1);
     const int i = gy * F.W + gx;
-    vf bq[NQ], xk[NQ], ps[9]; PxCoef c;
+    vf ps[9]; PxCoef c;
     if (valid) {
         c = px_coef<NINE>(F, gy, gx);
         if (coarse) {
@@ -372,52 +396,61 @@
 #pragma unroll
             for (int k = 0; k < 9; ++k) ps[k] = pp[k];
         }
-#pragma unroll
-        for (int q = 0; q < NQ; ++q) { bq[q] = (vf)b[(size_t)q * F.n + i]; xk[q] = X0 ? x1[(size_t)q * F.n + i] : bq[q] * c.dinv; s_a[q * LN + p] = xk[q]; }
-    }
-    if (nact == 0) return;
-    __syncthreads();
-#pragma unroll
-    for (int k = 1 - S0; k < MG_NS; ++k) {
-        vf* src = ((k + S0) & 1) ? s_a : s_b; vf* dst = ((k + S0) & 1) ? s_b : s_a;
-        if (ring(k + S0)) {
-            vf y[NQ]; lds_op<NQ, LW, LN, NINE>(c, src, p, xk, y);
-#pragma unroll
-            for (int q = 0; q < NQ; ++q) {
-                xk[q] = xk[q] + (bq[q] - y[q]) * (k == 0 ? c.dinv : c.dinv * mg_rk(k));
-                dst[q * LN + p] = xk[q];
-                if (k == MG_NS - 1 && interior) x[(size_t)q * F.n + i] = xk[q];
-            }
-        }
-        __syncthreads();
-    }
-    vf* xs = ((MG_NS + S0) & 1) ? s_a : s_b; vf* rs = ((MG_NS + S0) & 1) ? s_b : s_a;
-    if (ring(MG_NS + S0)) {
-        vf yv[NQ]; lds_op<NQ, LW, LN, NINE>(c, xs, p, xk, yv);
-#pragma unroll
-        for (int q = 0; q < NQ; ++q) rs[q * LN + p] = bq[q] - yv[q];
-    }
-    __syncthreads();
-    if (coarse) {
-        const bool xr = (c.ex & 1u) != 0, xl = (c.ex & 2u) != 0, yd = (c.ex & 4u) != 0, yu = (c.ex & 8u) != 0;
-        const bool in[9] = {xl && yu, yu, xr && yu, xl, true, xr, xl && yd, yd, xr && yd};
-        vf acc[NQ];
-#pragma unroll
-        for (int q = 0; q < NQ; ++q) acc[q] = 0.0f;
-#pragma unroll
-        for (int k = 0; k < 9; ++k)
-            if (in[k]) {
-#pragma unroll
-                for (int q = 0; q < NQ; ++q) acc[q] += ps[k] * rs[q * LN + p + (k / 3 - 1) * LW + (k % 3 - 1)];
-            }
-#pragma unroll
-        for (int q = 0; q < NQ; ++q) bc[(size_t)q * C.n + (gy >> 1) * C.W + (gx >> 1)] = acc[q];
-    }
+    }
+    const unsigned am = act_mask<NQ>(abit);
+    if (am == 0) return;
+    int qm[NQ]; act_list<NQ>(am, qm);
+    auto leg = [&](auto na_c) __attribute__((always_inline)) {
+        constexpr int NA = decltype(na_c)::value;
+        vf bq[NA], xk[NA];
+        if (valid) {
+#pragma unroll
+            for (int j = 0; j < NA; ++j) { const size_t o = (size_t)qm[j] * F.n + i; bq[j] = (vf)b[o]; xk[j] = X0 ? x1[o] : bq[j] * c.dinv; s_a[j * LN + p] = xk[j]; }
+        }
+        __syncthreads();
+#pragma unroll
+        for (int k = 1 - S0; k < MG_NS; ++k) {
+            vf* src = ((k + S0) & 1) ? s_a : s_b; vf* dst = ((k + S0) & 1) ? s_b : s_a;
+            if (ring(k + S0)) {
+                vf y[NA]; lds_op<NA, LW, LN, NINE>(c, src, p, xk, y);
+#pragma unroll
+                for (int j = 0; j < NA; ++j) {
+                    xk[j] = xk[j] + (bq[j] - y[j]) * (k == 0 ? c.dinv : c.dinv * mg_rk(k));
+                    dst[j * LN + p] = xk[j];
+                    if (k == MG_NS - 1 && interior) x[(size_t)qm[j] * F.n + i] = xk[j];
+                }
+            }
+            __syncthreads();
+        }
+        vf* xs = ((MG_NS + S0) & 1) ? s_a : s_b; vf* rs = ((MG_NS + S0) & 1) ? s_b : s_a;
+        if (ring(MG_NS + S0)) {
+            vf yv[NA]; lds_op<NA, LW, LN, NINE>(c, xs, p, xk, yv);
+#pragma unroll
+            for (int j = 0; j < NA; ++j) rs[j * LN + p] = bq[j] - yv[j];
+        }
+        __syncthreads();
+        if (coarse) {
+            const bool xr = (c.ex & 1u) != 0, xl = (c.ex & 2u) != 0, yd = (c.ex & 4u) != 0, yu = (c.ex & 8u) != 0;
+            const bool in[9] = {xl && yu, yu, xr && yu, xl, true, xr, xl && yd, yd, xr && yd};
+            vf acc[NA];
+#pragma unroll
+            for (int j = 0; j < NA; ++j) acc[j] = 0.0f;
+#pragma unroll
+            for (int k = 0; k < 9; ++k)
+                if (in[k]) {
+#pragma unroll
+                    for (int j = 0; j < NA; ++j) acc[j] += ps[k] * rs[j * LN + p + (k / 3 - 1) * LW + (k % 3 - 1)];
+                }
+#pragma unroll
+            for (int j = 0; j < NA; ++j) bc[(size_t)qm[j] * C.n + (gy >> 1) * C.W + (gx >> 1)] = acc[j];
+        }
+    };
+    act_dispatch<NQ>(__builtin_popcount(am), leg);
 }
 template <int NQ, int TX, int TY, typename TB, bool NINE>
 __global__ __launch_bounds__(mg_threads(TX, TY)) void k_mg_up(const PState* __restrict__ st, Lvl L, const TB* __restrict__ b, const vf* __restrict__ x, int Wc, int nc,
                                                               const vf* __restrict__ ec, vf* __restrict__ xo) {
-    const int nact = st->nactive;
+    int abit[NQ]; act_load<NQ>(st, abit);
     constexpr bool ODD = (MG_NS & 1) != 0;
     constexpr int HA = ODD ? MG_NS + 1 : MG_NS, HB = ODD ? MG_NS : MG_NS + 1, LW = TX + HA + HB, LH = TY + HA + HB, LN = LW * LH;
     constexpr int OL = ODD ? 1 : 0, OR = ODD ? 0 : 1;
@@ -431,56 +464,65 @@
     auto ring = [&](int k) { return valid && lx >= OL + k && lx <= LW - 1 - OR - k && ly >= OL + k && ly <= LH - 1 - OR - k; };
     const bool oy = (gy & 1) != 0, ox = (gx & 1) != 0;
     const int i = gy * L.W + gx;
-    vf bq[NQ], xk[NQ], pw[4]; PxCoef c;
+    vf pw[4]; PxCoef c;
     if (valid) {
         c = px_coef<NINE>(L, gy, gx);
 #pragma unroll
         for (int k = 0; k < 4; ++k) pw[k] = L.fpw[(size_t)k * L.n + i];
-#pragma unroll
-        for (int q = 0; q < NQ; ++q) { bq[q] = (vf)b[(size_t)q * L.n + i]; xk[q] = x[(size_t)q * L.n + i]; }
-        if (!oy && !ox) {
-            const int ip = (gy >> 1) * Wc + (gx >> 1);
-#pragma unroll
-            for (int q = 0; q < NQ; ++q) s_a[q * LN + p] = ec[(size_t)q * nc + ip];
-        }
-    }
-    if (nact == 0) return;
-    __syncthreads();
-    if (ring(0)) {
-        const bool xr = (c.ex & 1u) != 0, yd = (c.ex & 4u) != 0;
-        const int o0 = -(oy ? LW : 0) - (ox ? 1 : 0);
-        const int o1 = (oy && ox) ? -LW + 1 : (ox ? 1 : LW);
-        const bool e1 = (oy && ox) ? xr : (ox ? xr : yd);
-        const bool e2 = oy && ox && yd, e3 = oy && ox && yd && xr;
-        const bool copy = !oy && !ox;
-        const int a1 = e1 ? o1 : o0, a2 = e2 ? LW - 1 : o0, a3 = e3 ? LW + 1 : o0;
-        vf v0[NQ], v1[NQ], v2[NQ], v3[NQ];
-#pragma unroll
-        for (int q = 0; q < NQ; ++q) { v0[q] = s_a[q * LN + p + (copy ? 0 : o0)]; v1[q] = s_a[q * LN + p + (copy ? 0 : a1)]; v2[q] = s_a[q * LN + p + (copy ? 0 : a2)]; v3[q] = s_a[q * LN + p + (copy ? 0 : a3)]; }
-#pragma unroll
-        for (int q = 0; q < NQ; ++q) {
-            vf e = pw[0] * v0[q];
-            e = e1 ? e + pw[1] * v1[q] : e;
-            e = e2 ? e + pw[2] * v2[q] : e;
-            e = e3 ? e + pw[3] * v3[q] : e;
-            e = copy ? v0[q] : e;
-            xk[q] = xk[q] + e; s_b[q * LN + p] = xk[q];
-        }
-    }
-    __syncthreads();
-#pragma unroll
-    for (int k = 0; k < MG_NS; ++k) {
-        vf* src = (k & 1) ? s_a : s_b; vf* dst = (k & 1) ? s_b : s_a;
-        if (ring(k + 1)) {
-            vf y[NQ]; lds_op<NQ, LW, LN, NINE>(c, src, p, xk, y);
-#pragma unroll
-            for (int q = 0; q < NQ; ++q) {
-                xk[q] = xk[q] + (bq[q] - y[q]) * (k == 0 ? c.dinv : c.dinv * mg_rk(k));
-                if (k == MG_NS - 1) xo[(size_t)q * L.n + i] = xk[q]; else dst[q * LN + p] = xk[q];
-            }
-        }
-        if (k < MG_NS - 1) __syncthreads();
-    }
+    }
+    const unsigned am = act_mask<NQ>(abit);
+    if (am == 0) return;
+    int qm[NQ]; act_list<NQ>(am, qm);
+    auto leg = [&](auto na_c) __attribute__((always_inline)) {
+        constexpr int NA = decltype(na_c)::value;
+        vf bq[NA], xk[NA];
+        if (valid) {
+#pragma unroll
+            for (int j = 0; j < NA; ++j) { const size_t o = (size_t)qm[j] * L.n + i; bq[j] = (vf)b[o]; xk[j] = x[o]; }
+            if (!oy && !ox) {
+                const int ip = (gy >> 1) * Wc + (gx >> 1);
+#pragma unroll
+                for (int j = 0; j < NA; ++j) s_a[j * LN + p] = ec[(size_t)qm[j] * nc + ip];
+            }
+        }
+        __syncthreads();
+        if (ring(0)) {
+            const bool xr = (c.ex & 1u) != 0, yd = (c.ex & 4u) != 0;
+            const int o0 = -(oy ? LW : 0) - (ox ? 1 : 0);
+            const int o1 = (oy && ox) ? -LW + 1 : (ox ? 1 : LW);
+            const bool e1 = (oy && ox) ? xr : (ox ? xr : yd);
+            const bool e2 = oy && ox && yd, e3 = oy && ox && yd && xr;
+            const bool copy = !oy && !ox;
+            const int a1 = e1 ? o1 : o0, a2 = e2 ? LW - 1 : o0, a3 = e3 ? LW + 1 : o0;
+            vf v0[NA], v1[NA], v2[NA], v3[NA];
+#pragma unroll
+            for (int j = 0; j < NA; ++j) { v0[j] = s_a[j * LN + p + (copy ? 0 : o0)]; v1[j] = s_a[j * LN + p + (copy ? 0 : a1)]; v2[j] = s_a[j * LN + p + (copy ? 0 : a2)]; v3[j] = s_a[j * LN + p + (copy ? 0 : a3)]; }
+#pragma unroll
+            for (int j = 0; j < NA; ++j) {
+                vf e = pw[0] * v0[j];
+                e = e1 ? e + pw[1] * v1[j] : e;
+                e = e2 ? e + pw[2] * v2[j] : e;
+                e = e3 ? e + pw[3] * v3[j] : e;
+                e = copy ? v0[j] : e;
+                xk[j] = xk[j] + e; s_b[j * LN + p] = xk[j];
+            }
+        }
+        __syncthreads();
+#pragma unroll
+        for (int k = 0; k < MG_NS; ++k) {
+            vf* src = (k & 1) ? s_a : s_b; vf* dst = (k & 1) ? s_b : s_a;
+            if (ring(k + 1)) {
+                vf y[NA]; lds_op<NA, LW, LN, NINE>(c, src, p, xk, y);
+#pragma unroll
+                for (int j = 0; j < NA; ++j) {
+                    xk[j] = xk[j] + (bq[j] - y[j]) * (k == 0 ? c.dinv : c.dinv * mg_rk(k));
+                    if (k == MG_NS - 1) xo[(size_t)qm[j] * L.n + i] = xk[j]; else dst[j * LN + p] = xk[j];
+                }
+            }
+            if (k < MG_NS - 1) __syncthreads();
+        }
+    };
+    act_dispatch<NQ>(__builtin_popcount(am), leg);
 }
 constexpr int LBX = 32, LBY = 16, LBP = LBX + 1, LBN = LBY * LBP + 1;
 constexpr float LINE_OM = 0.9f;
@@ -551,7 +593,7 @@
 }
 template <int NQ, bool POST>
 __global__ __launch_bounds__(LBX * LBY, 8) void k_mg_block(const PState* __restrict__ st, Lvl L, const vf* __restrict__ b, const vf* __restrict__ xin, vf* __restrict__ xout) {
-    const int nact = st->nactive;
+    int abit[NQ]; act_load<NQ>(st, abit);
     constexpr int XW = LBX + 2, XN = XW * (LBY + 2);
     static_assert(NQ * XN <= (NQ + 6) * LBN, "the halo tile of the iterate lives where e1 and the factors go afterwards");
     __shared__ vf s_all[(2 * NQ + 6) * LBN];
@@ -564,71 +606,78 @@
     const int p = threadIdx.x, ly = p / LBX, lx = p - ly * LBX, gy = y0 + ly, gx = x0 + lx;
     const bool valid = ly < bh && lx < bw;
     const int i = gy * W + gx, lp = ly * LBP + lx;
-    vf own[NQ], bq[NQ];
-    if (POST) {
-        for (int h = p; h < XN; h += LBX * LBY) {
-            const int hy = h / XW, hx = h - hy * XW, yy = y0 + hy - 1, xx = x0 + hx - 1;
-            if (yy >= 0 && yy < H && xx >= 0 && xx < W) {
-#pragma unroll
-                for (int q = 0; q < NQ; ++q) s_x[q * XN + h] = xin[(size_t)q * L.n + yy * W + xx];
-            }
-        }
-    }
     vf fE_own = 0.f, fS_own = 0.f, c_xm = 0.f, c_xp = 0.f, c_ym = 0.f, c_yp = 0.f;
-    if (valid) {
-        c_xm = L.lxm[i]; c_xp = L.lxp[i]; c_ym = L.lym[i]; c_yp = L.lyp[i]; fE_own = L.fE[i]; fS_own = L.fS[i];
-#pragma unroll
-        for (int q = 0; q < NQ; ++q) bq[q] = b[(size_t)q * L.n + i];
-    }
-    if (nact == 0) return;
-    if (POST) {
-        __syncthreads();
+    if (valid) { c_xm = L.lxm[i]; c_xp = L.lxp[i]; c_ym = L.lym[i]; c_yp = L.lyp[i]; fE_own = L.fE[i]; fS_own = L.fS[i]; }
+    const unsigned am = act_mask<NQ>(abit);
+    if (am == 0) return;
+    {
+        auto on = [&](int q) { return ((am >> q) & 1u) != 0; };
+        vf own[NQ], bq[NQ];
+        if (POST) {
+            for (int h = p; h < XN; h += LBX * LBY) {
+                const int hy = h / XW, hx = h - hy * XW, yy = y0 + hy - 1, xx = x0 + hx - 1;
+                if (yy >= 0 && yy < H && xx >= 0 && xx < W) {
+#pragma unroll
+                    for (int q = 0; q < NQ; ++q) if (on(q)) s_x[q * XN + h] = xin[(size_t)q * L.n + yy * W + xx];
+                }
+            }
+        }
         if (valid) {
-            const vf d = L.fd[i];
-            const bool xr = gx + 1 < W, xl = gx > 0, yd = gy + 1 < H, yu = gy > 0;
-            const vf wW = xl ? L.fE[i - 1] : 0.f, wN = yu ? L.fS[i - W] : 0.f;
-            const int hp = (ly + 1) * XW + lx + 1;
+#pragma unroll
+            for (int q = 0; q < NQ; ++q) if (on(q)) bq[q] = b[(size_t)q * L.n + i];
+        }
+        if (POST) {
+            __syncthreads();
+            if (valid) {
+                const vf d = L.fd[i];
+                const bool xr = gx + 1 < W, xl = gx > 0, yd = gy + 1 < H, yu = gy > 0;
+                const vf wW = xl ? L.fE[i - 1] : 0.f, wN = yu ? L.fS[i - W] : 0.f;
+                const int hp = (ly + 1) * XW + lx + 1;
+#pragma unroll
+                for (int q = 0; q < NQ; ++q) {
+                    if (!on(q)) continue;
+                    own[q] = s_x[q * XN + hp];
+                    const vf vE = s_x[q * XN + hp + 1], vW = s_x[q * XN + hp - 1], vS = s_x[q * XN + hp + XW], vN = s_x[q * XN + hp - XW];
+                    vf y = d * own[q];
+                    y = xr ? y - fE_own * vE : y;
+                    y = xl ? y - wW * vW : y;
+                    y = yd ? y - fS_own * vS : y;
+                    y = yu ? y - wN * vN : y;
+                    bq[q] = bq[q] - y;
+                }
+            }
+            __syncthreads();
+        }
+        if (valid) {
+            s_xm[lp] = c_xm; s_xp[lp] = c_xp; s_ym[lp] = c_ym; s_yp[lp] = c_yp; s_xw[lp] = fE_own; s_yw[lp] = fS_own;
+#pragma unroll
+            for (int q = 0; q < NQ; ++q) if (on(q)) s_r[q * LBN + lp] = bq[q];
+        }
+        __syncthreads();
+        if (!POST) { if (p < LBY * NQ) { const int row = p % LBY, q = p / LBY; if (row < bh && on(q)) { const int o = row * LBP; line_solve<LBX, 1>(s_r + q * LBN + o, s_e1 + q * LBN + o, s_xm + o, s_xp + o, s_xw + o, bw); } } }
+        else       { if (p < LBX * NQ) { const int col = p % LBX, q = p / LBX; if (col < bw && on(q)) line_solve<LBY, LBP>(s_r + q * LBN + col, s_e1 + q * LBN + col, s_ym + col, s_yp + col, s_yw + col, bh); } }
+        __syncthreads();
+        if (valid) {
 #pragma unroll
             for (int q = 0; q < NQ; ++q) {
-                own[q] = s_x[q * XN + hp];
-                const vf vE = s_x[q * XN + hp + 1], vW = s_x[q * XN + hp - 1], vS = s_x[q * XN + hp + XW], vN = s_x[q * XN + hp - XW];
-                vf y = d * own[q];
-                y = xr ? y - fE_own * vE : y;
-                y = xl ? y - wW * vW : y;
-                y = yd ? y - fS_own * vS : y;
-                y = yu ? y - wN * vN : y;
-                bq[q] = bq[q] - y;
-            }
-        }
-        __syncthreads();
-    }
-    if (valid) {
-        s_xm[lp] = c_xm; s_xp[lp] = c_xp; s_ym[lp] = c_ym; s_yp[lp] = c_yp; s_xw[lp] = fE_own; s_yw[lp] = fS_own;
-#pragma unroll
-        for (int q = 0; q < NQ; ++q) s_r[q * LBN + lp] = bq[q];
-    }
-    __syncthreads();
-    if (!POST) { if (p < LBY * NQ) { const int row = p % LBY, q = p / LBY; if (row < bh) { const int o = row * LBP; line_solve<LBX, 1>(s_r + q * LBN + o, s_e1 + q * LBN + o, s_xm + o, s_xp + o, s_xw + o, bw); } } }
-    else       { if (p < LBX * NQ) { const int col = p % LBX, q = p / LBX; if (col < bw) line_solve<LBY, LBP>(s_r + q * LBN + col, s_e1 + q * LBN + col, s_ym + col, s_yp + col, s_yw + col, bh); } }
-    __syncthreads();
-    if (valid) {
-#pragma unroll
-        for (int q = 0; q < NQ; ++q) {
-            vf acc = 0.0f;
-            if (!POST) { if (ly + 1 < bh) acc += fS_own * s_e1[q * LBN + lp + LBP]; if (ly > 0) acc += s_yw[lp - LBP] * s_e1[q * LBN + lp - LBP]; }
-            else       { if (lx + 1 < bw) acc += fE_own * s_e1[q * LBN + lp + 1];   if (lx > 0) acc += s_xw[lp - 1] * s_e1[q * LBN + lp - 1]; }
-            s_r[q * LBN + lp] = acc;
-        }
-    }
-    __syncthreads();
-    if (!POST) { if (p < LBX * NQ) { const int col = p % LBX, q = p / LBX; if (col < bw) line_solve<LBY, LBP>(s_r + q * LBN + col, s_r + q * LBN + col, s_ym + col, s_yp + col, s_yw + col, bh); } }
-    else       { if (p < LBY * NQ) { const int row = p % LBY, q = p / LBY; if (row < bh) { const int o = row * LBP; line_solve<LBX, 1>(s_r + q * LBN + o, s_r + q * LBN + o, s_xm + o, s_xp + o, s_xw + o, bw); } } }
-    __syncthreads();
-    if (valid) {
-#pragma unroll
-        for (int q = 0; q < NQ; ++q) {
-            const vf u = (s_e1[q * LBN + lp] + s_r[q * LBN + lp]) * LINE_OM;
-            xout[(size_t)q * L.n + i] = POST ? own[q] + u : u;
+                if (!on(q)) continue;
+                vf acc = 0.0f;
+                if (!POST) { if (ly + 1 < bh) acc += fS_own * s_e1[q * LBN + lp + LBP]; if (ly > 0) acc += s_yw[lp - LBP] * s_e1[q * LBN + lp - LBP]; }
+                else       { if (lx + 1 < bw) acc += fE_own * s_e1[q * LBN + lp + 1];   if (lx > 0) acc += s_xw[lp - 1] * s_e1[q * LBN + lp - 1]; }
+                s_r[q * LBN + lp] = acc;
+            }
+        }
+        __syncthreads();
+        if (!POST) { if (p < LBX * NQ) { const int col = p % LBX, q = p / LBX; if (col < bw && on(q)) line_solve<LBY, LBP>(s_r + q * LBN + col, s_r + q * LBN + col, s_ym + col, s_yp + col, s_yw + col, bh); } }
+        else       { if (p < LBY * NQ) { const int row = p % LBY, q = p / LBY; if (row < bh && on(q)) { const int o = row * LBP; line_solve<LBX, 1>(s_r + q * LBN + o, s_r + q * LBN + o, s_xm + o, s_xp + o, s_xw + o, bw); } } }
+        __syncthreads();
+        if (valid) {
+#pragma unroll
+            for (int q = 0; q < NQ; ++q) {
+                if (!on(q)) continue;
+                const vf u = (s_e1[q * LBN + lp] + s_r[q * LBN + lp]) * LINE_OM;
+                xout[(size_t)q * L.n + i] = POST ? own[q] + u : u;
+            }
         }
     }
 }
@@ -816,14 +865,13 @@
 }
 template <int P0>
 __global__ __launch_bounds__(MID_T) void k_mg_mid(const PState* __restrict__ st, MidPack P, int sweeps) {
-    const int nact = st->nactive;
     __shared__ vf sA[MID_T * P0], sB[MID_T * P0], sC[MID_N1], sS[MID_STASH];
     const int q = blockIdx.x, t = threadIdx.x;
+    if (st->active[q] == 0) return;
     const Lvl& L0 = P.lv[0];
     vf b[P0];
 #pragma unroll
     for (int k = 0; k < P0; ++k) { const int i = t + k * MID_T; b[k] = i < L0.n ? L0.b[(size_t)q * L0.n + i] : 0.f; }
-    if (nact == 0) return;
     mid_level<P0, 0>(P, q, t, sA, sB, sC, sS, b, sweeps);
 }
 
@@ -866,86 +914,116 @@
 template <int NQ>
 __global__ __launch_bounds__(256) void k_cg_apply(const PState* __restrict__ st, Lvl L, const vf* __restrict__ z, const double* __restrict__ r,
                                                   double* __restrict__ w, double* __restrict__ partial) {
-    const int nact = st->nactive;
+    int abit[NQ]; act_load<NQ>(st, abit);
     const int lb = mg_tile_of_block(blockIdx.x, gridDim.x);
     const int i = lb * 256 + threadIdx.x;
-    double acc[3 * NQ];
-#pragma unroll
-    for (int q = 0; q < 3 * NQ; ++q) acc[q] = 0.0;
+    double acc[2 * NQ];
+#pragma unroll
+    for (int q = 0; q < 2 * NQ; ++q) acc[q] = 0.0;
     auto uv = [&](int j, int q) { return (double)z[(size_t)q * L.n + j]; };
     double y[NQ], rq[NQ], uq[NQ];
 #pragma unroll
     for (int q = 0; q < NQ; ++q) { y[q] = 0.0; rq[q] = 0.0; uq[q] = 0.0; }
     if (i < L.n) {
-        lvl_op<NQ>(L, i, uv, y);
-#pragma unroll
-        for (int q = 0; q < NQ; ++q) { rq[q] = r[(size_t)q * L.n + i]; uq[q] = uv(i, q); }
-    }
-    if (nact == 0) return;
+        lvl_op<NQ>(L, i, uv, y, abit);
+#pragma unroll
+        for (int q = 0; q < NQ; ++q) if (abit[q]) { rq[q] = r[(size_t)q * L.n + i]; uq[q] = uv(i, q); }
+    }
+    if (act_mask<NQ>(abit) == 0) return;
     if (i < L.n) {
 #pragma unroll
         for (int q = 0; q < NQ; ++q) {
+            if (!abit[q]) continue;
             const double u = uq[q], rv = rq[q];
             w[(size_t)q * L.n + i] = y[q];
-            acc[q] = rv * u; acc[NQ + q] = y[q] * u; acc[2 * NQ + q] = rv * rv;
-        }
-    }
-    mg_block_reduce<3 * NQ>(acc, partial, lb);
+            acc[q] = rv * u; acc[NQ + q] = y[q] * u;
+        }
+    }
+    mg_block_reduce<2 * NQ>(acc, partial, lb);
 }
 template <int NQ>
 __global__ void k_cg_fin(const PState* __restrict__ st, const double* __restrict__ partial, int nb, double* __restrict__ sums) {
-    if (st->nactive == 0) return;
-    double s[NQ]; mg_final_reduce_strided<NQ>(partial + blockIdx.x * NQ, nb, 3 * NQ, s);
-    if (threadIdx.x < NQ) sums[blockIdx.x * NQ + threadIdx.x] = s[threadIdx.x];
+    int abit[NQ]; act_load<NQ>(st, abit);
+    if (act_mask<NQ>(abit) == 0) return;
+    double s[NQ]; mg_final_reduce_strided<NQ>(partial + blockIdx.x * NQ, nb, 2 * NQ, s, abit);
+#pragma unroll
+    for (int q = 0; q < NQ; ++q) if (threadIdx.x == q) sums[blockIdx.x * NQ + q] = s[q];
 }
 template <int NQ>
-__global__ __launch_bounds__(256) void k_cg_update(int n, const PState* __restrict__ sc, PState* __restrict__ sn, const double* __restrict__ sums, double rtol2, int first,
+__global__ __launch_bounds__(256) void k_cg_update(int n, const PState* __restrict__ sc, PState* __restrict__ sn, const double* __restrict__ sums, int first,
                                                    const vf* __restrict__ z, const double* __restrict__ w, double* __restrict__ p, double* __restrict__ s,
-                                                   double* __restrict__ x, double* __restrict__ r, vf* __restrict__ rf, PState* __restrict__ host_out, int seq) {
-    if (sc->nactive == 0) { if (blockIdx.x == 0 && threadIdx.x == 0) { *sn = *sc; if (host_out) pcg_publish(host_out, *sc, seq); } return; }
+                                                   double* __restrict__ x, double* __restrict__ r, vf* __restrict__ rf, double* __restrict__ partial_rho) {
+    int abit[NQ]; act_load<NQ>(sc, abit);
+    if (act_mask<NQ>(abit) == 0) return;
     double al[NQ], be[NQ]; bool act[NQ];
 #pragma unroll
     for (int q = 0; q < NQ; ++q) {
-        const double gam = sums[q], del = sums[NQ + q], rho = sums[2 * NQ + q];
-        act[q] = sc->active[q] != 0 && rho > rtol2 * sc->bb[q];
+        act[q] = abit[q] != 0; al[q] = 0.0; be[q] = 0.0;
+        if (!act[q]) continue;
+        const double gam = sums[q], del = sums[NQ + q];
         be[q] = first ? 0.0 : gam / sc->gam[q];
         al[q] = first ? gam / del : gam / (del - be[q] * gam / sc->alp[q]);
     }
     if (blockIdx.x == 0 && threadIdx.x == 0) {
-        int na = 0;
 #pragma unroll
         for (int q = 0; q < NQ; ++q) {
             sn->bb[q] = sc->bb[q];
             sn->gam[q] = act[q] ? sums[q] : sc->gam[q]; sn->alp[q] = act[q] ? al[q] : sc->alp[q];
-            sn->iters[q] = sc->iters[q] + (act[q] ? 1 : 0); sn->active[q] = act[q] ? 1 : 0; na += act[q] ? 1 : 0;
-            sn->rho[q] = sc->active[q] != 0 ? sums[2 * NQ + q] : sc->rho[q];
-        }
+            sn->iters[q] = sc->iters[q] + (act[q] ? 1 : 0);
+        }
+    }
+    const int i = blockIdx.x * 256 + threadIdx.x;
+    double acc[NQ];
+#pragma unroll
+    for (int q = 0; q < NQ; ++q) acc[q] = 0.0;
+    if (i < n) {
+        vf zq[NQ]; double wq[NQ], pq[NQ], sq[NQ], xq[NQ], rq[NQ];
+#pragma unroll
+        for (int q = 0; q < NQ; ++q) {
+            zq[q] = 0.f; wq[q] = pq[q] = sq[q] = xq[q] = rq[q] = 0.0;
+            if (act[q]) {
+                const size_t j = (size_t)q * n + i;
+                zq[q] = z[j]; wq[q] = w[j]; xq[q] = x[j]; rq[q] = r[j];
+                if (!first) { pq[q] = p[j]; sq[q] = s[j]; }
+            }
+        }
+#pragma unroll
+        for (int q = 0; q < NQ; ++q) {
+            if (!act[q]) continue;
+            const size_t j = (size_t)q * n + i;
+            const double zv = (double)zq[q], wv = wq[q];
+            const double pn = first ? zv : zv + be[q] * pq[q];
+            const double sv = first ? wv : wv + be[q] * sq[q];
+            p[j] = pn; s[j] = sv;
+            x[j] = xq[q] + al[q] * pn;
+            const double rn = rq[q] - al[q] * sv;
+            r[j] = rn; rf[j] = (vf)rn;
+            acc[q] = rn * rn;
+        }
+    }
+    mg_block_reduce<NQ>(acc, partial_rho);
+}
+template <int NQ>
+__global__ __launch_bounds__(256) void k_cg_next(const PState* __restrict__ sc, PState* __restrict__ sn, const double* __restrict__ partial_rho, int nb, double rtol2,
+                                                 PState* __restrict__ host_out, int seq) {
+    int abit[NQ]; act_load<NQ>(sc, abit);
+    if (act_mask<NQ>(abit) == 0) {
+        if (threadIdx.x == 0) { *sn = *sc; if (host_out) pcg_publish(host_out, *sc, seq); }
+        return;
+    }
+    double s[NQ]; mg_final_reduce_strided<NQ>(partial_rho, nb, NQ, s, abit);
+#pragma unroll
+    for (int q = 0; q < NQ; ++q)
+        if (threadIdx.x == q) {
+            sn->active[q] = (abit[q] != 0 && s[q] > rtol2 * sc->bb[q]) ? 1 : 0;
+            sn->rho[q] = abit[q] != 0 ? s[q] : sc->rho[q];
+        }
+    __syncthreads();
+    if (threadIdx.x == 0) {
+        int na = 0;
+        for (int q = 0; q < NQ; ++q) na += sn->active[q];
         sn->nactive = na;
         if (host_out) pcg_publish(host_out, *sn, seq);
-    }
-    const int i = blockIdx.x * 256 + threadIdx.x;
-    if (i >= n) return;
-    vf zq[NQ]; double wq[NQ], pq[NQ], sq[NQ], xq[NQ], rq[NQ];
-#pragma unroll
-    for (int q = 0; q < NQ; ++q) {
-        zq[q] = 0.f; wq[q] = pq[q] = sq[q] = xq[q] = rq[q] = 0.0;
-        if (act[q]) {
-            const size_t j = (size_t)q * n + i;
-            zq[q] = z[j]; wq[q] = w[j]; xq[q] = x[j]; rq[q] = r[j];
-            if (!first) { pq[q] = p[j]; sq[q] = s[j]; }
-        }
-    }
-#pragma unroll
-    for (int q = 0; q < NQ; ++q) {
-        if (!act[q]) continue;
-        const size_t j = (size_t)q * n + i;
-        const double zv = (double)zq[q], wv = wq[q];
-        const double pn = first ? zv : zv + be[q] * pq[q];
-        const double sv = first ? wv : wv + be[q] * sq[q];
-        p[j] = pn; s[j] = sv;
-        x[j] = xq[q] + al[q] * pn;
-        const double rn = rq[q] - al[q] * sv;
-        r[j] = rn; rf[j] = (vf)rn;
     }
 }
 template <int NQ>
@@ -988,6 +1066,7 @@
     const Lvl& F = lv[0];
     const int N = F.n, nb = cdiv(N, 256);
     double *x6 = B.x6, *r = B.r, *p = B.p, *sv = B.sv, *w = B.w, *partial = B.partial, *sums = B.sums;
+    double* partial_rho = partial + (size_t)nb * 2 * NQ;
     vf* rf = B.rf;
     PState* st = B.st;
     const PState* cur = st;
@@ -1078,11 +1157,12 @@
         NCT_TRY(kt_b(NCT_KT_WLS_APPLY));
         hipLaunchKernelGGL(k_cg_apply<NQ>, dim3(nb), dim3(256), 0, s, cur, F, z, (const double*)r, (double*)w, (double*)partial); LCHK();
         NCT_TRY(kt_e());
-        hipLaunchKernelGGL(k_cg_fin<NQ>, dim3(3), dim3(256), 0, s, cur, (const double*)partial, nb, (double*)sums); LCHK();
+        hipLaunchKernelGGL(k_cg_fin<NQ>, dim3(2), dim3(256), 0, s, cur, (const double*)partial, nb, (double*)sums); LCHK();
         NCT_TRY(kt_b(NCT_KT_WLS_UPDATE));
-        hipLaunchKernelGGL(k_cg_update<NQ>, dim3(nb), dim3(256), 0, s, N, cur, nxt, (const double*)sums, rtol2, it == 0 ? 1 : 0, z, (const double*)w,
-                           (double*)p, (double*)sv, (double*)x6, (double*)r, rf, pub_to, pub_seq); LCHK();
+        hipLaunchKernelGGL(k_cg_update<NQ>, dim3(nb), dim3(256), 0, s, N, cur, nxt, (const double*)sums, it == 0 ? 1 : 0, z, (const double*)w,
+                           (double*)p, (double*)sv, (double*)x6, (double*)r, rf, partial_rho); LCHK();
         NCT_TRY(kt_e());
+        hipLaunchKernelGGL(k_cg_next<NQ>, dim3(1), dim3(256), 0, s, cur, nxt, (const double*)partial_rho, nb, rtol2, pub_to, pub_seq); LCHK();
         cur = nxt;
         return 0;
     };
@@ -1132,7 +1212,7 @@
         if (fin.nactive == 0) { done = true; break; }
         if (it >= maxit && seen == issued) break;
         if (B.forecast) {
-            const int ridx = its_seen > 0 ? its_seen - 1 : 0;
+            const int ridx = its_seen;
             int need = -1; bool ok = prev_its >= 0 && ridx > prev_its;
             if (ok) {
                 need = 1;
@@ -1142,7 +1222,7 @@
                     if (!(rho > 0.0) || !(prev_rho[q] > 0.0) || !(thr > 0.0)) { ok = false; break; }
                     const double decay = pow(rho / prev_rho[q], 1.0 / (double)(ridx - prev_its));
                     if (!(decay < 0.95)) { ok = false; break; }
-                    const double m = rho * decay <= thr ? 1.0 : 1.0 + ceil(log(thr / (rho * decay)) / log(decay));
+                    const double m = ceil(log(thr / rho) / log(decay));
                     if (m > need) need = (int)(m < 1e6 ? m : 1e6);
                 }
             }
@@ -1156,7 +1236,10 @@
     for (int q = 0; q < NQ; ++q) B.iters[q] = fin.iters[q];
     if (B.trace) {
         int mx = 0; for (int q = 0; q < NQ; ++q) mx = fin.iters[q] > mx ? fin.iters[q] : mx;
-        fprintf(stderr, "nct wls: %d x %d, %d iterations enqueued, %d needed (+1 that finds every system converged), %d snapshots read\n", F.W, F.H, it, mx, seen + 1);
+        int sum = 0; for (int q = 0; q < NQ; ++q) sum += fin.iters[q];
+        fprintf(stderr, "nct wls: %d x %d, %d iterations enqueued, %d needed (%d system-passes of %d), %d snapshots read, per system:", F.W, F.H, it, mx, sum, NQ * mx, seen + 1);
+        for (int q = 0; q < NQ; ++q) fprintf(stderr, " %d", fin.iters[q]);
+        fprintf(stderr, "\n");
     }
     return 0;
 }
```

Result: no change. 15.77, median of 6 (+0.3%).
